# Patryk27/strolle

Hardware: AMD Instinct MI355X
Metric: Mray/s (primary + shadow + GI rays traced per second, whole job) (higher is better)
Workload: dtype f32

## Files before the change

include/strolle_hip.h:

```cpp
#ifndef STROLLE_HIP_H
#define STROLLE_HIP_H

#include <stddef.h>
#include <stdint.h>

#ifdef __cplusplus
extern "C" {
#endif

typedef struct StEngine StEngine;
typedef uint64_t StHandle;

enum StStatus {
    ST_OK = 0,
    ST_ERR_INVALID_ARGUMENT = 1,
    ST_ERR_NO_DEVICE = 2,
    ST_ERR_UNKNOWN_CAMERA = 3,
    ST_ERR_EMPTY_MESH = 4,
    ST_ERR_HIP = 5,
    ST_ERR_ATLAS_FULL = 6,
    ST_ERR_IO = 7,
    ST_ERR_PARSE = 8,
    ST_ERR_UNSUPPORTED = 9,
    ST_ERR_BVH_TOO_DEEP = 10,
// ... 400 lines not shown
int st_dist_shutdown(StEngine* e);
int st_dist_rank(StEngine* e, int* rank, int* world);
int st_dist_set_partition(StEngine* e, StHandle camera, uint32_t cols, uint32_t apron, StDistRect* owned, StDistRect* window);
int st_dist_set_grid(StEngine* e, StHandle camera, const StDistGrid* grid, uint32_t apron, StDistRect* owned, StDistRect* window);
int st_dist_gather(StEngine* e, StHandle camera, const void* frame, void* full_on_root, void* hip_stream);
int st_dist_wait(StEngine* e, StHandle camera, const void* frame, void* hip_stream, int host_wait);
int st_dist_gather_ms(StEngine* e, StHandle camera, float* ms);

enum StOutputFormat { ST_FORMAT_RGBA32F = 0, ST_FORMAT_RGBA16F = 1, ST_FORMAT_RGBA8_UNORM_SRGB = 2, ST_FORMAT_BGRA8_UNORM_SRGB = 3 };
int st_camera_set_output_format(StEngine* e, StHandle camera, int format);

typedef struct StTuning {
    uint32_t struct_size;
    uint32_t overlap;
    uint32_t fuse;
    uint32_t fuse_di_head;
    uint32_t fuse_spatial;
    uint32_t fuse_gi_sampling;
    uint32_t fuse_gi_validation;
    uint32_t fuse_gi_reprojection;
    uint32_t fuse_wavelet;
    uint32_t fuse_compose;
    uint32_t preview_both;
    uint32_t variance_in_reproject;
    uint32_t lean_frame;
    uint32_t skip_scratch_stores;
    uint32_t di_head_on_main;
    uint32_t alias_gi_history;
    uint32_t tile_map;
    uint32_t tile_map_denoise;
    int32_t side_priority;
    uint32_t staging;
    uint32_t double_buffer;
    uint32_t packed_base;
    uint32_t tick_timing;
    uint32_t anyhit_fast;
    uint32_t compact_bvh;
    uint32_t allow_deep_bvh;
    uint32_t device_bake;
    uint32_t wide_bvh;
    uint32_t wide_stack_entries;
    uint32_t primary_packets;
    uint32_t side_start;
} StTuning;
int st_engine_get_tuning(StEngine* e, StTuning* out);
int st_engine_set_tuning(StEngine* e, const StTuning* tuning);

enum StArithmetic { ST_ARITH_FAST = 0, ST_ARITH_EXACT = 1 };
int st_engine_set_arithmetic(StEngine* e, int arithmetic);
int st_engine_get_arithmetic(StEngine* e, int* out);

enum StBufferId {
    ST_BUF_PRIM_GBUFFER_D0_A = 0, ST_BUF_PRIM_GBUFFER_D0_B = 1, ST_BUF_PRIM_GBUFFER_D1_A = 2, ST_BUF_PRIM_GBUFFER_D1_B = 3,
    ST_BUF_PRIM_SURFACE_MAP_A = 4, ST_BUF_PRIM_SURFACE_MAP_B = 5, ST_BUF_REPROJECTION_MAP = 6, ST_BUF_VELOCITY_MAP = 7,
    ST_BUF_DI_RESERVOIRS_0 = 8, ST_BUF_DI_RESERVOIRS_1 = 9, ST_BUF_DI_RESERVOIRS_2 = 10,
    ST_BUF_DI_DIFF_SAMPLES = 11, ST_BUF_DI_DIFF_PREV_COLORS = 12, ST_BUF_DI_DIFF_CURR_COLORS = 13,
    ST_BUF_DI_DIFF_MOMENTS_A = 14, ST_BUF_DI_DIFF_MOMENTS_B = 15, ST_BUF_DI_DIFF_STASH = 16, ST_BUF_DI_SPEC_SAMPLES = 17,
    ST_BUF_GI_D0 = 18, ST_BUF_GI_D1 = 19, ST_BUF_GI_D2 = 20,
    ST_BUF_GI_RESERVOIRS_0 = 21, ST_BUF_GI_RESERVOIRS_1 = 22, ST_BUF_GI_RESERVOIRS_2 = 23, ST_BUF_GI_RESERVOIRS_3 = 24,
    ST_BUF_GI_DIFF_SAMPLES = 25, ST_BUF_GI_DIFF_PREV_COLORS = 26, ST_BUF_GI_DIFF_CURR_COLORS = 27,
    ST_BUF_GI_DIFF_MOMENTS_A = 28, ST_BUF_GI_DIFF_MOMENTS_B = 29, ST_BUF_GI_DIFF_STASH = 30, ST_BUF_GI_SPEC_SAMPLES = 31,
    ST_BUF_REF_HITS = 32, ST_BUF_REF_RAYS = 33, ST_BUF_REF_COLORS = 34,
    ST_BUF_DBG_USED_MEMORY = 35,
    ST_BUF_COUNT = 36
};
int st_camera_read_buffer(StEngine* e, StHandle camera, int buffer_id, void* out, size_t capacity, size_t* written);
int st_camera_write_buffer(StEngine* e, StHandle camera, int buffer_id, const void* data, size_t bytes);
int st_debug_keep_all_planes(StEngine* e, int keep);
int st_camera_buffer_stale(StEngine* e, StHandle camera, int buffer_id, int* stale);
enum StPassBit {
    ST_PASS_PRIM_VISIBILITY = 1u << 0, ST_PASS_FRAME_REPROJECTION = 1u << 1,
    ST_PASS_DI_SAMPLING = 1u << 2, ST_PASS_DI_TEMPORAL = 1u << 3, ST_PASS_DI_SPATIAL_PICK = 1u << 4, ST_PASS_DI_SPATIAL_TRACE = 1u << 5,
    ST_PASS_DI_SPATIAL_SAMPLE = 1u << 6, ST_PASS_DI_RESOLVING = 1u << 7,
    ST_PASS_GI_REPROJECTION = 1u << 8, ST_PASS_GI_SAMPLING_A = 1u << 9, ST_PASS_GI_SAMPLING_B = 1u << 10, ST_PASS_GI_TEMPORAL = 1u << 11,
    ST_PASS_GI_SPATIAL_PICK = 1u << 12, ST_PASS_GI_SPATIAL_TRACE = 1u << 13, ST_PASS_GI_SPATIAL_SAMPLE = 1u << 14,
    ST_PASS_GI_PREVIEW_0 = 1u << 15, ST_PASS_GI_PREVIEW_1 = 1u << 16, ST_PASS_GI_RESOLVING = 1u << 17,
    ST_PASS_DENOISE_REPROJECT_DI = 1u << 18, ST_PASS_DENOISE_REPROJECT_GI = 1u << 19, ST_PASS_DENOISE_VARIANCE = 1u << 20,
    ST_PASS_DENOISE_WAVELET_0 = 1u << 21,
    ST_PASS_COMPOSITION = 1u << 26, ST_PASS_BVH_HEATMAP = 1u << 27, ST_PASS_REF_TRACING = 1u << 28, ST_PASS_REF_SHADING = 1u << 29,
    ST_PASS_POST = 1u << 30
};
int st_debug_set_pass_mask(StEngine* e, uint64_t mask);
int st_debug_set_launch_filter(StEngine* e, uint64_t filter);
int st_debug_variance_flags(StEngine* e, StHandle camera, uint64_t* tile_mask_out, size_t capacity_tiles, size_t* tiles);
int st_debug_last_launches(StEngine* e, uint64_t* out_bits, size_t capacity, size_t* count);
int st_camera_ray_count(StEngine* e, StHandle camera, uint64_t* out, int reset);
int st_debug_read_scene(StEngine* e, int what, void* out, size_t capacity, size_t* written);
int st_debug_world(StEngine* e, uint32_t* light_count, uint32_t* next_frame);
int st_debug_image_rect(StEngine* e, StHandle id, uint32_t out_xywh[4]);
int st_debug_bvh_refresh(StEngine* e, uint64_t* primitives, uint64_t* reused);
int st_debug_read_lut(StEngine* e, int what, float* out, size_t capacity_floats, size_t* written_floats);

enum { ST_GLTF_OVERRIDE_REFLECTANCE = 1, ST_GLTF_OVERRIDE_PERCEPTUAL_ROUGHNESS = 2 };
typedef struct StGltfOptions {
    StHandle first_handle;
    StHandle first_image_handle;
    uint32_t override_mask;
    float reflectance;
    float perceptual_roughness;
    uint32_t subdivide;
    float light_radius;
    uint32_t _pad;
} StGltfOptions;
typedef struct StGltfSummary {
    uint32_t meshes, triangles, materials, images;
    uint32_t images_dropped;
    uint32_t primitives_skipped;
    uint32_t lights;
    uint32_t lights_skipped;
} StGltfSummary;
int st_scene_load_gltf(StEngine* e, const char* path, const StGltfOptions* options, StGltfSummary* summary);
int st_scene_load_gltf_memory(StEngine* e, const void* bytes, size_t size, const char* base_dir, const StGltfOptions* options, StGltfSummary* summary);
int st_decode_png(const void* bytes, size_t size, uint8_t* out_rgba, size_t capacity, uint32_t* width, uint32_t* height);
int st_decode_image(const void* bytes, size_t size, uint8_t* out_rgba, size_t capacity, uint32_t* width, uint32_t* height);

int st_debug_copy_bandwidth(StEngine* e, size_t bytes, int iters, double* out_gbps);

enum { ST_PROFILE_TIMING = 1, ST_PROFILE_TRAVERSAL_BYTES = 2,
       ST_PROFILE_GROUP_ATROUS = 4 ,
       ST_PROFILE_KERNEL_EVENTS = 8  };
enum { ST_PROFILE_MAX_KERNELS = 64 };
typedef struct StKernelProfile {
    char name[48];
    uint32_t launches;
    float total_ms;
    double algorithmic_bytes;
    double traversal_bytes;
} StKernelProfile;
int st_profile_enable(StEngine* e, int enabled);
int st_profile_read(StEngine* e, StKernelProfile* out, size_t capacity, size_t* count, int reset);

#ifdef __cplusplus
}
#endif
#endif
```

rust/strolle-hip/src/ffi.rs:

```rust
#![allow(non_camel_case_types, dead_code)]
use std::ffi::c_void;
use std::os::raw::c_char;

#[repr(C)]
#[derive(Clone, Copy, Default)]
pub struct StMeshTriangle {
    pub positions: [[f32; 3]; 3],
    pub normals: [[f32; 3]; 3],
    pub uvs: [[f32; 2]; 3],
    pub tangents: [[f32; 4]; 3],
}

#[repr(C)]
#[derive(Clone, Copy, Default)]
pub struct StMaterial {
    pub base_color: [f32; 4],
    pub emissive: [f32; 4],
    pub perceptual_roughness: f32,
    pub metallic: f32,
    pub reflectance: f32,
    pub ior: f32,
    pub base_color_texture: u64,
    pub emissive_texture: u64,
    pub metallic_roughness_texture: u64,
// ... 62 lines not shown
    pub alias_gi_history: u32,
    pub tile_map: u32,
    pub tile_map_denoise: u32,
    pub side_priority: i32,
    pub staging: u32,
    pub double_buffer: u32,
    pub packed_base: u32,
    pub tick_timing: u32,
    pub anyhit_fast: u32,
    pub compact_bvh: u32,
    pub allow_deep_bvh: u32,
    pub device_bake: u32,
    pub wide_bvh: u32,
    pub wide_stack_entries: u32,
    pub primary_packets: u32,
    pub side_start: u32,
}

#[repr(C)]
#[derive(Clone, Copy, PartialEq, Eq, Debug)]
pub struct StDistGrid {
    pub cols: u32,
    pub rows: u32,
    pub row_edge: [u32; 17],
    pub col_edge: [[u32; 17]; 16],
}

#[repr(C)]
#[derive(Clone, Copy, Default, PartialEq, Eq, Debug)]
pub struct StDistRect {
    pub x0: u32,
    pub y0: u32,
    pub x1: u32,
    pub y1: u32,
}

#[repr(C)]
#[derive(Clone, Copy)]
pub struct StDistUniqueId {
    pub internal: [c_char; 128],
}

pub enum StEngine {}

pub const ST_RAY_COHERENT: u32 = 1;
pub const ST_RAY_MAPPED_NORMAL: u32 = 2;

extern "C" {
    pub fn st_engine_create(device_ordinal: i32, out: *mut *mut StEngine) -> i32;
    pub fn st_engine_destroy(e: *mut StEngine);
    pub fn st_last_error() -> *const c_char;
    pub fn st_build_commit() -> *const c_char;
    pub fn st_mesh_insert(e: *mut StEngine, id: u64, triangles: *const StMeshTriangle, count: usize) -> i32;
    pub fn st_mesh_remove(e: *mut StEngine, id: u64) -> i32;
    pub fn st_material_insert(e: *mut StEngine, id: u64, material: *const StMaterial) -> i32;
    pub fn st_material_has(e: *mut StEngine, id: u64) -> i32;
    pub fn st_material_remove(e: *mut StEngine, id: u64) -> i32;
    pub fn st_image_insert_rgba8(e: *mut StEngine, id: u64, w: u32, h: u32, rgba: *const u8, srgb: i32) -> i32;
    pub fn st_image_insert_device_rgba8(e: *mut StEngine, id: u64, w: u32, h: u32, device_rgba: *const c_void, row_pitch: usize, is_dynamic: i32) -> i32;
    pub fn st_image_remove(e: *mut StEngine, id: u64) -> i32;
    pub fn st_instance_insert(e: *mut StEngine, id: u64, mesh: u64, material: u64, xform12: *const f32) -> i32;
    pub fn st_instance_remove(e: *mut StEngine, id: u64) -> i32;
    pub fn st_light_insert(e: *mut StEngine, id: u64, light: *const StLight) -> i32;
    pub fn st_light_remove(e: *mut StEngine, id: u64) -> i32;
    pub fn st_sun_update(e: *mut StEngine, azimuth: f32, altitude: f32) -> i32;
    pub fn st_camera_create(e: *mut StEngine, camera: *const StCamera, out: *mut u64) -> i32;
    pub fn st_camera_update(e: *mut StEngine, camera: u64, desc: *const StCamera) -> i32;
    pub fn st_camera_delete(e: *mut StEngine, camera: u64) -> i32;
    pub fn st_camera_set_output_format(e: *mut StEngine, camera: u64, format: i32) -> i32;
    pub fn st_tick(e: *mut StEngine, hip_stream: *mut c_void) -> i32;
    pub fn st_render_camera(e: *mut StEngine, camera: u64, out_device: *mut c_void, hip_stream: *mut c_void) -> i32;
    pub fn st_camera_present_copy(e: *mut StEngine, camera: u64, src_device: *const c_void, dst_host: *mut c_void, bytes: usize, hip_stream: *mut c_void) -> i32;
    pub fn st_camera_present_ready(e: *mut StEngine, camera: u64, dst_host: *const c_void, wait: i32, ready: *mut i32) -> i32;
    pub fn st_set_seed(e: *mut StEngine, seed: u64) -> i32;
    pub fn st_set_blue_noise(e: *mut StEngine, rgba: *const u8, bytes: usize) -> i32;
    pub fn st_engine_set_arithmetic(e: *mut StEngine, arithmetic: i32) -> i32;
    pub fn st_set_bvh_refresh(e: *mut StEngine, mode: i32) -> i32;
    pub fn st_debug_walk_overflow(e: *mut StEngine, overflows: *mut u64, wide_stack_entries: *mut u32, packets_off: *mut u32) -> i32;
    pub fn st_debug_auto_tree(e: *mut StEngine, leaf_run_weight: *mut f32, first_tree_on_device: *mut u32) -> i32;
    pub fn st_debug_device_builds(e: *mut StEngine, ticks: *mut u64) -> i32;
    pub fn st_debug_device_tree_refits(e: *mut StEngine, ticks: *mut u64) -> i32;
    pub fn st_engine_get_tuning(e: *mut StEngine, out: *mut StTuning) -> i32;
    pub fn st_engine_set_tuning(e: *mut StEngine, tuning: *const StTuning) -> i32;
    pub fn st_camera_set_window(e: *mut StEngine, camera: u64, x0: u32, y0: u32, x1: u32, y1: u32) -> i32;
    pub fn st_dist_partition(width: u32, height: u32, world: u32, cols: u32, rank: u32, owned: *mut StDistRect) -> i32;
    pub fn st_dist_window(width: u32, height: u32, owned: *const StDistRect, apron: u32, window: *mut StDistRect) -> i32;
    pub fn st_dist_unique_id(out: *mut StDistUniqueId) -> i32;
    pub fn st_dist_init(e: *mut StEngine, rank: i32, world: i32, id: *const StDistUniqueId) -> i32;
    pub fn st_dist_shutdown(e: *mut StEngine) -> i32;
    pub fn st_dist_set_partition(e: *mut StEngine, camera: u64, cols: u32, apron: u32, owned: *mut StDistRect, window: *mut StDistRect) -> i32;
    pub fn st_dist_grid(width: u32, height: u32, world: u32, cols: u32, out: *mut StDistGrid) -> i32;
    pub fn st_dist_grid_tile(grid: *const StDistGrid, rank: u32, owned: *mut StDistRect) -> i32;
    pub fn st_dist_grid_rebalance(width: u32, height: u32, current: *const StDistGrid, tile_cost: *const f32, max_step: u32, out: *mut StDistGrid) -> i32;
    pub fn st_dist_set_grid(e: *mut StEngine, camera: u64, grid: *const StDistGrid, apron: u32, owned: *mut StDistRect, window: *mut StDistRect) -> i32;
    pub fn st_dist_gather(e: *mut StEngine, camera: u64, frame: *const c_void, full_on_root: *mut c_void, hip_stream: *mut c_void) -> i32;
    pub fn st_dist_wait(e: *mut StEngine, camera: u64, frame: *const c_void, hip_stream: *mut c_void, host_wait: i32) -> i32;
}

pub const ST_ENV_KEEP_SUN: u32 = 1;
pub const ST_ENV_UNIFORM_SAMPLING: u32 = 2;
#[repr(C)]
#[derive(Clone, Copy, Debug, Default)]
pub struct StEnvironmentDesc {
    pub struct_size: u32,
    pub flags: u32,
    pub intensity: f32,
    pub yaw: f32,
}
extern "C" {
    pub fn st_environment_set(e: *mut StEngine, texels: *const f32, width: u32, height: u32, channels: u32, desc: *const StEnvironmentDesc) -> i32;
    pub fn st_environment_set_device(e: *mut StEngine, texels_device: *const c_void, width: u32, height: u32, channels: u32, row_pitch_bytes: usize, desc: *const StEnvironmentDesc) -> i32;
    pub fn st_environment_update(e: *mut StEngine, desc: *const StEnvironmentDesc) -> i32;
    pub fn st_environment_clear(e: *mut StEngine) -> i32;
    pub fn st_decode_hdr(bytes: *const c_void, size: usize, out_rgb: *mut f32, capacity_floats: usize, width: *mut u32, height: *mut u32) -> i32;
    pub fn st_debug_environment_eval(e: *mut StEngine, dirs_device: *const f32, n: u32, rgb_device: *mut f32, hip_stream: *mut c_void) -> i32;
    pub fn st_debug_environment_sample(e: *mut StEngine, u_device: *const f32 , n: u32, dir_pdf_device: *mut f32, hip_stream: *mut c_void) -> i32;
    pub fn st_debug_environment_pdf(e: *mut StEngine, dirs_device: *const f32, n: u32, pdf_device: *mut f32, hip_stream: *mut c_void) -> i32;
    pub fn st_debug_environment_sanitized(e: *mut StEngine, texels: *mut u64) -> i32;
    pub fn st_debug_environment_table(e: *mut StEngine, table: *mut c_void, capacity_bytes: usize, cells_x: *mut u32, cells_y: *mut u32) -> i32;
}

pub const ST_TONEMAP_NONE: u32 = 0;
pub const ST_TONEMAP_REINHARD: u32 = 1;
pub const ST_TONEMAP_REINHARD_LUMINANCE: u32 = 2;
pub const ST_TONEMAP_ACES_FITTED: u32 = 3;
pub const ST_TONEMAP_PBR_NEUTRAL: u32 = 4;
pub const ST_DISPLAY_AUTO_EXPOSURE: u32 = 1;
#[repr(C)]
#[derive(Clone, Copy, Debug, Default)]
pub struct StDisplayDesc {
    pub struct_size: u32,
    pub tonemap: u32,
    pub flags: u32,
    pub exposure_ev: f32,
    pub ev_min: f32,
    pub ev_max: f32,
    pub low_fraction: f32,
    pub high_fraction: f32,
    pub max_ev_step_up: f32,
    pub max_ev_step_down: f32,
}
extern "C" {
    pub fn st_camera_set_display(e: *mut StEngine, camera: u64, desc: *const StDisplayDesc) -> i32;
    pub fn st_camera_get_display(e: *mut StEngine, camera: u64, out: *mut StDisplayDesc, enabled: *mut i32) -> i32;
    pub fn st_camera_exposure(e: *mut StEngine, camera: u64, scale: *mut f32, metered_ev: *mut f32, adapted_ev: *mut f32) -> i32;
    pub fn st_debug_camera_histogram(e: *mut StEngine, camera: u64, bins: *mut u32) -> i32;
}

extern "C" {
    pub fn st_engine_set_deformation_motion(e: *mut StEngine, enabled: i32) -> i32;
    pub fn st_engine_get_deformation_motion(e: *mut StEngine, enabled: *mut i32) -> i32;
    pub fn st_engine_set_normal_mapping(e: *mut StEngine, enabled: i32) -> i32;
    pub fn st_engine_get_normal_mapping(e: *mut StEngine, enabled: *mut i32) -> i32;
    pub fn st_debug_deformation(e: *mut StEngine, instances_with_previous: *mut u64, previous_bytes: *mut u64) -> i32;
}

#[repr(C)]
#[derive(Clone, Copy, Debug, Default)]
pub struct StMorphDelta {
    pub position: [f32; 3],
    pub normal: [f32; 3],
}
extern "C" {
    pub fn st_mesh_set_morph_targets(e: *mut StEngine, mesh: u64, deltas: *const StMorphDelta, corner_count: usize, target_count: u32) -> i32;
    pub fn st_instance_set_morph_weights(e: *mut StEngine, instance: u64, weights: *const f32, target_count: u32) -> i32;
    pub fn st_debug_morphing(e: *mut StEngine, ticks: *mut u64, triangles: *mut u64, delta_bytes: *mut u64) -> i32;
// ... 272 lines not shown
```

strolle_amd/api.py:

```python
from __future__ import annotations

import ctypes as C
import dataclasses
import enum
import math
import os
import sys
from typing import Optional, Sequence

import numpy as np

_HERE = os.path.dirname(os.path.abspath(__file__))
LIB_PATH = os.environ.get("STROLLE_HIP_LIB") or os.path.join(_HERE, "csrc", "libstrolle_hip.so")
if os.environ.get("STROLLE_HIP_LIB"):
    LIB_PATH = os.environ["STROLLE_HIP_LIB"]


class StMeshTriangle(C.Structure):
    _fields_ = [("positions", C.c_float * 9), ("normals", C.c_float * 9), ("uvs", C.c_float * 6), ("tangents", C.c_float * 12)]


class StSkinVertex(C.Structure):
    _fields_ = [("joints", C.c_uint16 * 4), ("weights", C.c_float * 4)]

# ... 624 lines not shown
            self.environment_set_device = fn("environment_set_device", [vp, vp, u32, u32, u32, sz, P(StEnvironmentDesc)])
            self.environment_update = fn("environment_update", [vp, P(StEnvironmentDesc)])
            self.environment_clear = fn("environment_clear", [vp])
            self.debug_environment_eval = fn("debug_environment_eval", [vp, vp, u32, vp, vp])
            self.debug_environment_sample = fn("debug_environment_sample", [vp, vp, u32, vp, vp])
            self.debug_environment_pdf = fn("debug_environment_pdf", [vp, vp, u32, vp, vp])
            self.debug_environment_sanitized = fn("debug_environment_sanitized", [vp, P(u64)])
            self.debug_environment_table = fn("debug_environment_table", [vp, vp, sz, P(u32), P(u32)])
        if hasattr(lib, prefix + "camera_set_display"):
            self.camera_set_display = fn("camera_set_display", [vp, u64, P(StDisplayDesc)])
            self.camera_get_display = fn("camera_get_display", [vp, u64, P(StDisplayDesc), P(i32)])
            self.camera_exposure = fn("camera_exposure", [vp, u64, P(C.c_float), P(C.c_float), P(C.c_float)])
            self.debug_camera_histogram = fn("debug_camera_histogram", [vp, u64, P(u32)])
        if hasattr(lib, prefix + "camera_set_post"):
            self.camera_set_post = fn("camera_set_post", [vp, u64, P(StPostDesc)])
            self.camera_get_post = fn("camera_get_post", [vp, u64, P(StPostDesc), P(i32)])
            self.camera_output_size = fn("camera_output_size", [vp, u64, P(u32), P(u32)])
            self.post_process = fn("post_process", [vp, P(StPostDesc), vp, u32, u32, vp, i32, vp])
        if hasattr(lib, prefix + "camera_set_upscale"):
            self.camera_set_upscale = fn("camera_set_upscale", [vp, u64, P(StUpscaleDesc)])
            self.camera_get_upscale = fn("camera_get_upscale", [vp, u64, P(StUpscaleDesc), P(i32)])
            self.upscale_process = fn("upscale_process", [vp, P(StUpscaleDesc), vp, u32, u32, vp, i32, vp])
            self.debug_set_upscale_fused = fn("debug_set_upscale_fused", [vp, i32])
        if hasattr(lib, prefix + "camera_set_bloom"):
            self.camera_set_bloom = fn("camera_set_bloom", [vp, u64, P(StBloomDesc)])
            self.camera_get_bloom = fn("camera_get_bloom", [vp, u64, P(StBloomDesc), P(i32)])
            self.bloom_plan = fn("bloom_plan", [P(StBloomDesc), u32, u32, P(u32), P(u32), P(C.c_float)])
            self.debug_set_bloom_tail = fn("debug_set_bloom_tail", [vp, i32, P(u32)])
            self.bloom_process = fn("bloom_process", [vp, P(StBloomDesc), P(StDisplayDesc), vp, u32, u32, vp, i32, vp])
        if hasattr(lib, prefix + "camera_set_motion_blur"):
            self.camera_set_motion_blur = fn("camera_set_motion_blur", [vp, u64, P(StMotionBlurDesc)])
            self.camera_get_motion_blur = fn("camera_get_motion_blur", [vp, u64, P(StMotionBlurDesc), P(i32)])
            self.motion_blur_process = fn("motion_blur_process", [vp, P(StMotionBlurDesc), P(StDisplayDesc), vp, vp, vp, u32, u32, vp, i32, vp])
        if hasattr(lib, prefix + "camera_set_dof"):
            self.camera_set_dof = fn("camera_set_dof", [vp, u64, P(StDofDesc)])
            self.camera_get_dof = fn("camera_get_dof", [vp, u64, P(StDofDesc), P(i32)])
            self.dof_plan = fn("dof_plan", [P(StDofDesc), u32, u32, P(u32), P(u32), P(C.c_float)])
            self.dof_process = fn("dof_process", [vp, P(StDofDesc), P(StDisplayDesc), P(C.c_float), vp, vp, u32, u32, vp, i32, vp])
        if hasattr(lib, prefix + "camera_set_fog"):
            self.camera_set_fog = fn("camera_set_fog", [vp, u64, P(StFogDesc)])
            self.camera_get_fog = fn("camera_get_fog", [vp, u64, P(StFogDesc), P(i32)])
            self.fog_process = fn("fog_process", [vp, P(StFogDesc), P(StDisplayDesc), P(C.c_float), P(C.c_float), vp, vp, u32, u32, vp, i32, vp])
        if hasattr(lib, prefix + "camera_set_lens"):
            self.camera_set_lens = fn("camera_set_lens", [vp, u64, P(StLensDesc)])
            self.camera_get_lens = fn("camera_get_lens", [vp, u64, P(StLensDesc), P(i32)])
            self.lens_plan = fn("lens_plan", [P(StLensDesc), u32, u32, P(StLensPlan)])
            self.lens_process = fn("lens_process", [vp, P(StLensDesc), P(StDisplayDesc), vp, u32, u32, vp, i32, vp])
            self.debug_set_lens_gather = fn("debug_set_lens_gather", [vp, i32])
        if hasattr(lib, prefix + "camera_set_color_grading"):
            self.camera_set_color_grading = fn("camera_set_color_grading", [vp, u64, P(StColorGradingDesc)])
            self.camera_get_color_grading = fn("camera_get_color_grading", [vp, u64, P(StColorGradingDesc), P(i32)])
            self.color_grading_plan = fn("color_grading_plan", [P(StColorGradingDesc), P(StColorGradingPlan)])
            self.color_grading_process = fn("color_grading_process", [vp, P(StColorGradingDesc), P(StDisplayDesc), vp, u32, vp, u32, u32, vp, i32, vp])
            self.lut_insert = fn("lut_insert", [vp, u64, u32, P(C.c_float)]); self.lut_remove = fn("lut_remove", [vp, u64])
        if hasattr(lib, prefix + "camera_set_light_shafts"):
            self.camera_set_light_shafts = fn("camera_set_light_shafts", [vp, u64, P(StLightShaftsDesc)])
            self.camera_get_light_shafts = fn("camera_get_light_shafts", [vp, u64, P(StLightShaftsDesc), P(i32)])
            self.light_shafts_process = fn("light_shafts_process", [vp, P(StLightShaftsDesc), P(StDisplayDesc), P(C.c_float), P(C.c_float), vp, vp, u32, u32, vp, i32, vp])
        if hasattr(lib, prefix + "mesh_set_skin"):
            self.mesh_set_skin = fn("mesh_set_skin", [vp, u64, vp, sz, u32])
        if hasattr(lib, prefix + "mesh_set_morph_targets"):
            self.mesh_set_morph_targets = fn("mesh_set_morph_targets", [vp, u64, vp, sz, u32])
            self.instance_set_morph_weights = fn("instance_set_morph_weights", [vp, u64, P(C.c_float), u32])
            self.debug_morphing = fn("debug_morphing", [vp, P(u64), P(u64), P(u64)])
        if hasattr(lib, prefix + "engine_set_deformation_motion"):
            self.engine_set_deformation_motion = fn("engine_set_deformation_motion", [vp, i32])
            self.engine_get_deformation_motion = fn("engine_get_deformation_motion", [vp, P(i32)])
            self.debug_deformation = fn("debug_deformation", [vp, P(u64), P(u64)])
        if hasattr(lib, prefix + "engine_set_normal_mapping"):
            self.engine_set_normal_mapping = fn("engine_set_normal_mapping", [vp, i32])
            self.engine_get_normal_mapping = fn("engine_get_normal_mapping", [vp, P(i32)])
        if has_device:
            self.camera_set_rows = fn("camera_set_rows", [vp, u64, u32, u32])
            self.camera_set_output_format = fn("camera_set_output_format", [vp, u64, i32])
            self.image_insert_device_rgba8 = fn("image_insert_device_rgba8", [vp, u64, u32, u32, vp, sz, i32])
            self.debug_bvh_refresh = fn("debug_bvh_refresh", [vp, P(u64), P(u64)])
            self.scene_load_gltf = fn("scene_load_gltf", [vp, C.c_char_p, P(StGltfOptions), P(StGltfSummary)])
            self.scene_load_gltf_memory = fn("scene_load_gltf_memory", [vp, vp, sz, C.c_char_p, P(StGltfOptions), P(StGltfSummary)])
            self.decode_png = fn("decode_png", [vp, sz, vp, sz, P(u32), P(u32)])
            self.engine_set_arithmetic = fn("engine_set_arithmetic", [vp, i32]); self.engine_get_arithmetic = fn("engine_get_arithmetic", [vp, P(i32)])
            self.camera_write_buffer = fn("camera_write_buffer", [vp, u64, i32, vp, sz])
            self.debug_set_pass_mask = fn("debug_set_pass_mask", [vp, u64]); self.debug_set_launch_filter = fn("debug_set_launch_filter", [vp, u64]); self.debug_last_launches = fn("debug_last_launches", [vp, P(u64), sz, P(sz)])
            self.debug_keep_all_planes = fn("debug_keep_all_planes", [vp, i32])
            self.camera_buffer_stale = fn("camera_buffer_stale", [vp, u64, i32, P(i32)])
            self.camera_present_copy = fn("camera_present_copy", [vp, u64, vp, vp, sz, vp])
            self.camera_present_ready = fn("camera_present_ready", [vp, u64, vp, i32, P(i32)])
            if hasattr(lib, prefix + "scene_trace_rays"):
                self.scene_trace_rays = fn("scene_trace_rays", [vp, vp, u32, vp, u32, vp])
                self.scene_occluded = fn("scene_occluded", [vp, vp, u32, vp, vp])
                self.camera_pick = fn("camera_pick", [vp, u64, vp, u32, vp, vp])
                self.scene_trace_rays_host = fn("scene_trace_rays_host", [vp, vp, u32, vp])
            if hasattr(lib, prefix + "camera_render_aovs"):
                self.camera_render_aovs = fn("camera_render_aovs", [vp, u64, P(StAovTargets), vp])
            if hasattr(lib, prefix + "instance_set_pose"):
                self.instance_set_pose = fn("instance_set_pose", [vp, u64, P(C.c_float), u32])
                self.debug_skinning = fn("debug_skinning", [vp, P(u64), P(u64), P(u64)])
                self.debug_read_posed = fn("debug_read_posed", [vp, u64, P(C.c_float), sz, P(sz)])
            self.profile_enable = fn("profile_enable", [vp, i32])
            self.profile_read = fn("profile_read", [vp, P(StKernelProfile), sz, P(sz), i32])
            self.last_error = getattr(lib, prefix + "last_error"); self.last_error.restype = C.c_char_p; self.last_error.argtypes = []


_STATUS = {1: "invalid argument", 2: "no HIP device (host-only engine or HIP unavailable)", 3: "camera does not exist",
           4: "mesh contains no triangles", 5: "HIP runtime error", 6: "no more space in the atlas", 7: "file could not be read",
           8: "malformed scene file", 9: "unsupported scene file feature",
           10: "the BVH is deeper than the kernels' traversal stack (the scene was uploaded; pushes beyond 24 pending entries are dropped)",
           11: "collective transport error"}
ST_ERR_BVH_TOO_DEEP = 10


class EngineBase:

    def __init__(self, binding: _Binding, device: int = 0):
        self._b = binding
        h = C.c_void_p()
        self._check(binding.engine_create(device, C.byref(h)) if binding.has_device else binding.engine_create(C.byref(h)))
        self._h = h
        self._keep = []

    def _check(self, status: int):
        if status != 0:
            detail = ""
            if self._b.has_device:
                msg = self._b.last_error()
                detail = f": {msg.decode(errors='replace')}" if msg else ""
            raise StrolleError(f"{_STATUS.get(status, 'error')} (status {status}){detail}")

    def close(self):
        if getattr(self, "_h", None):
            self._b.engine_destroy(self._h)
            self._h = None

    def __del__(self):
        try:
            self.close()
        except Exception:
            pass

    def insert_mesh(self, handle: int, mesh: Mesh):
        data = mesh.pack()
        self._check(self._b.mesh_insert(self._h, handle, data.ctypes.data, len(data)))

    def remove_mesh(self, handle: int):
        self._check(self._b.mesh_remove(self._h, handle))

    def set_skin(self, mesh: int, joints, weights, joint_count: int):
        joints = np.asarray(joints).reshape(-1, 4); weights = np.asarray(weights, np.float32).reshape(-1, 4)
        corners = np.zeros(len(joints), SKIN_VERTEX_DTYPE)
        corners["joints"] = joints; corners["weights"] = weights
        self._check(self._b.mesh_set_skin(self._h, mesh, corners.ctypes.data if len(corners) else None, len(corners), joint_count))

    def set_morph_targets(self, mesh: int, position_deltas, normal_deltas):
        dp = np.asarray(position_deltas, np.float32); dn = np.asarray(normal_deltas, np.float32)
        if dp.ndim != 4 or dp.shape[2:] != (3, 3) or dn.shape != dp.shape:
            raise StrolleError("morph deltas: expected two arrays of shape (K, n, 3, 3)")
        deltas = np.zeros((dp.shape[0], dp.shape[1] * 3), MORPH_DELTA_DTYPE)
        deltas["position"] = dp.reshape(dp.shape[0], -1, 3); deltas["normal"] = dn.reshape(dp.shape[0], -1, 3)
        self._check(self._b.mesh_set_morph_targets(self._h, mesh, deltas.ctypes.data if deltas.size else None, deltas.shape[1], deltas.shape[0]))

    def insert_material(self, handle: int, material: Material):
        m = material.to_c()
        self._check(self._b.material_insert(self._h, handle, C.byref(m)))

    def has_material(self, handle: int) -> bool:
        return bool(self._b.material_has(self._h, handle))

# ... 120 lines not shown
    def bvh_refits(self):
        a, b = C.c_uint64(), C.c_uint64()
        self._check(self._b.debug_bvh_refits(self._h, C.byref(a), C.byref(b)))
        return a.value, b.value

    def bvh_depth(self):
        if not hasattr(self._b, "debug_bvh_depth"):
            raise StrolleError("bvh_depth() is a seam of libstrolle_hip.so (st_debug_bvh_depth); this engine's library does not export it")
        a, b = C.c_uint32(), C.c_uint32()
        self._check(self._b.debug_bvh_depth(self._h, C.byref(a), C.byref(b)))
        return a.value, b.value

    def walk_overflow(self):
        n, entries, off = C.c_uint64(), C.c_uint32(), C.c_uint32()
        self._check(self._b.debug_walk_overflow(self._h, C.byref(n), C.byref(entries), C.byref(off)))
        return n.value, entries.value, off.value

    def auto_tree(self):
        w, d = C.c_float(), C.c_uint32()
        self._check(self._b.debug_auto_tree(self._h, C.byref(w), C.byref(d)))
        return float(w.value), bool(d.value)

    def image_rect(self, handle: int):
        r = (C.c_uint32 * 4)()
        self._check(self._b.debug_image_rect(self._h, handle, r))
        return tuple(r)

    def bvh_refresh(self):
        n, r = C.c_uint64(), C.c_uint64()
        self._check(self._b.debug_bvh_refresh(self._h, C.byref(n), C.byref(r)))
        return n.value, r.value


_lib_cache = {}


def load_library(path: str = LIB_PATH) -> C.CDLL:
    if path not in _lib_cache:
        if not os.path.exists(path):
            raise StrolleError(f"{path} is missing: run `python -c 'import __graft_entry__ as g; g.build()'` (no CPU fallback exists)")
        if os.environ.get("STROLLE_HIP_PRELOAD_TORCH") == "1" and "torch" not in sys.modules:
            import torch
        _lib_cache[path] = C.CDLL(path)
    return _lib_cache[path]


def library_build_commit(path: str = LIB_PATH) -> Optional[str]:
    lib = load_library(path)
    if not hasattr(lib, "st_build_commit"):
        return None
    lib.st_build_commit.restype = C.c_char_p
    return lib.st_build_commit().decode(errors="replace")


class Engine(EngineBase):

    def __init__(self, device: int = 0, exact: Optional[bool] = None):
        super().__init__(_Binding(load_library(), "st_", True), device)
        if exact is not None:
            self.set_exact(exact)

    def set_exact(self, exact: bool):
        self._check(self._b.engine_set_arithmetic(self._h, 1 if exact else 0))

    @property
    def exact(self) -> bool:
        out = C.c_int()
        self._check(self._b.engine_get_arithmetic(self._h, C.byref(out)))
        return out.value == 1

    def write_buffer(self, camera: int, buffer: "Buffer", data: np.ndarray):
        data = np.ascontiguousarray(data)
        self._check(self._b.camera_write_buffer(self._h, camera, int(buffer), data.ctypes.data, data.nbytes))

    def keep_all_planes(self, keep: bool):
        self._check(self._b.debug_keep_all_planes(self._h, 1 if keep else 0))

    def set_pass_mask(self, mask: int):
        self._check(self._b.debug_set_pass_mask(self._h, mask & 0xFFFFFFFFFFFFFFFF))

    def set_launch_filter(self, mask: int):
        self._check(self._b.debug_set_launch_filter(self._h, mask & 0xFFFFFFFFFFFFFFFF))

    def last_launches(self):
        arr = (C.c_uint64 * 64)(); n = C.c_size_t()
        self._check(self._b.debug_last_launches(self._h, arr, 64, C.byref(n)))
        return [arr[i] for i in range(min(n.value, 64))]

    def tick(self, stream: int = 0):
        self._check(self._b.tick(self._h, stream))

    def render_camera(self, handle: int, out_device_ptr: int = 0, stream: int = 0):
        self._check(self._b.render_camera(self._h, handle, out_device_ptr, stream))

    def trace_rays(self, rays_ptr: int, count: int, hits_ptr: int, coherent: bool = False, stream: int = 0, mapped_normal: bool = False):
        flags = (RAY_COHERENT if coherent else 0) | (RAY_MAPPED_NORMAL if mapped_normal else 0)
        self._check(self._b.scene_trace_rays(self._h, rays_ptr, count, hits_ptr, flags, stream))

    def occluded(self, rays_ptr: int, count: int, out_ptr: int, stream: int = 0):
        self._check(self._b.scene_occluded(self._h, rays_ptr, count, out_ptr, stream))

    def pick(self, camera: int, pixels_ptr: int, count: int, hits_ptr: int, stream: int = 0):
        self._check(self._b.camera_pick(self._h, camera, pixels_ptr, count, hits_ptr, stream))

    def render_aovs(self, camera: int, planes: dict, stream=None):
        t = StAovTargets(); t.struct_size = C.sizeof(StAovTargets)
        for k, v in planes.items():
            k = Aov(k)
            if v is None:
                continue
            if hasattr(v, "data_ptr"):
                scalar, comps = AOV_ELEMENT[k]
                per_pixel = v.shape[-1] if comps > 1 and v.dim() > 0 else comps
                if not v.is_contiguous() or v.element_size() != np.dtype(scalar).itemsize or per_pixel != comps:
                    raise StrolleError(f"AOV plane {k.name}: expected a contiguous tensor of {comps} x {np.dtype(scalar).name} per pixel")
                v = v.data_ptr()
            t.planes[int(k)] = int(v)
        if stream is not None and hasattr(stream, "cuda_stream"):
            stream = stream.cuda_stream
        self._check(self._b.camera_render_aovs(self._h, camera, C.byref(t), stream or 0))

    def set_pose(self, instance: int, matrices):
        if matrices is None:
            self._check(self._b.instance_set_pose(self._h, instance, None, 0)); return
        m = np.asarray(matrices, np.float32).reshape(-1, 3, 4)
        flat = np.ascontiguousarray(m.transpose(0, 2, 1).reshape(-1), dtype=np.float32)
        self._check(self._b.instance_set_pose(self._h, instance, flat.ctypes.data_as(C.POINTER(C.c_float)), len(m)))

    def set_morph_weights(self, instance: int, weights):
        if weights is None:
            self._check(self._b.instance_set_morph_weights(self._h, instance, None, 0)); return
        w = np.ascontiguousarray(np.asarray(weights, np.float32).reshape(-1))
        self._check(self._b.instance_set_morph_weights(self._h, instance, w.ctypes.data_as(C.POINTER(C.c_float)), len(w)))

    def morphing_stats(self):
        a, b, c = C.c_uint64(), C.c_uint64(), C.c_uint64()
        self._check(self._b.debug_morphing(self._h, C.byref(a), C.byref(b), C.byref(c)))
        return a.value, b.value, c.value

    def skinning_stats(self):
        a, b, c = C.c_uint64(), C.c_uint64(), C.c_uint64()
        self._check(self._b.debug_skinning(self._h, C.byref(a), C.byref(b), C.byref(c)))
        return a.value, b.value, c.value

    def read_posed(self, instance: int) -> np.ndarray:
        n = C.c_size_t()
        self._check(self._b.debug_read_posed(self._h, instance, None, 0, C.byref(n)))
        out = np.zeros(n.value, np.float32)
        self._check(self._b.debug_read_posed(self._h, instance, out.ctypes.data_as(C.POINTER(C.c_float)), n.value, C.byref(n)))
        return out.reshape(-1, 24)

    def set_deformation_motion(self, enabled: bool):
        self._check(self._b.engine_set_deformation_motion(self._h, 1 if enabled else 0))

    @property
    def deformation_motion(self) -> bool:
        on = C.c_int()
        self._check(self._b.engine_get_deformation_motion(self._h, C.byref(on)))
        return bool(on.value)

    def set_normal_mapping(self, enabled: bool):
        self._check(self._b.engine_set_normal_mapping(self._h, 1 if enabled else 0))

    def get_normal_mapping(self) -> bool:
        on = C.c_int()
        self._check(self._b.engine_get_normal_mapping(self._h, C.byref(on)))
# ... 461 lines not shown
```

strolle_amd/csrc/k_common.h:

```cpp
#pragma once
#include "st_device.h"
#include "st_passes.h"
#include "st_kernels.h"

namespace st {

constexpr int kBlockThreads = 256;
#ifdef ST_MIN_WAVES
#define ST_KERNEL_BOUNDS __launch_bounds__(kBlockThreads, ST_MIN_WAVES)
#else
#define ST_KERNEL_BOUNDS __launch_bounds__(kBlockThreads)
#endif
#define ST_STACK_LDS(SE, name) extern __shared__ __align__(16) unsigned char st_stack_lds_[]; SE* name = reinterpret_cast<SE*>(st_stack_lds_)
inline uint32_t stack_lds_bytes(const KArgs& a, size_t slot_bytes) { return a.stack_entries * (uint32_t)kBlockThreads * (uint32_t)slot_bytes; }

struct TileWindow { uint32_t tx0, tx1, ty0, ty1; };
__host__ __device__ inline TileWindow tile_window(const KArgs& a, bool half_x) {
    uint32_t tiles_x = (a.width + 7u) >> 3;
    if (half_x) tiles_x >>= 1;
    const uint32_t shift = half_x ? 4u : 3u, round = half_x ? 15u : 7u;
    TileWindow w;
    w.tx0 = a.col0 >> shift;
    w.tx1 = (a.col1 + round) >> shift; if (w.tx1 > tiles_x) w.tx1 = tiles_x;
    if (w.tx0 > w.tx1) w.tx0 = w.tx1;
    w.ty0 = a.row0 >> 3;
    w.ty1 = (a.row1 + 7u) >> 3;
    return w;
}
struct LaunchDims { uint32_t tiles_x, tile_x0, tile_y0, tile_y1, blocks; };
inline LaunchDims launch_dims(const KArgs& a, bool half_x) {
    const TileWindow w = tile_window(a, half_x);
    LaunchDims d;
    d.tiles_x = w.tx1 - w.tx0; d.tile_x0 = w.tx0;
    d.tile_y0 = w.ty0; d.tile_y1 = w.ty1;
    const uint32_t groups_x = (d.tiles_x + 3u) / 4u;
    d.blocks = groups_x * (d.tile_y1 - d.tile_y0);
    return d;
}

ST_D TileCoord resolve_tile(const KArgs& a, bool half_x) {
    const TileWindow w = tile_window(a, half_x);
    TileCoord tc = tile_for_thread(w.tx1 - w.tx0, w.ty1 - w.ty0, a.tile_map);
    tc.x += w.tx0; tc.y += w.ty0;
    return tc;
}
ST_D bool resolve_gid_of_block(const KArgs& a, bool half_x, uint32_t b, U2* gid) {
    const TileWindow w = tile_window(a, half_x);
    TileCoord tc = tile_for_block(b, w.tx1 - w.tx0, w.ty1 - w.ty0, a.tile_map);
    tc.x += w.tx0; tc.y += w.ty0;
    if (!tc.valid) return false;
    *gid = pixel_in_tile(tc);
    return true;
}
ST_D bool resolve_gid(const KArgs& a, bool half_x, U2* gid) {
    const TileCoord tc = resolve_tile(a, half_x);
    if (!tc.valid) return false;
    *gid = pixel_in_tile(tc);
    return true;
}
ST_D bool owns_pixel(const KArgs& a, U2 p) { return p.x < a.width && p.y < a.height && p.y >= a.row0 && p.y < a.row1 && p.x >= a.col0 && p.x < a.col1; }

constexpr uint32_t kStack16Texels = 4u * 65536u;
inline uint32_t stack16_limit(const KArgs& a) {
    if (a.bvh_w) return a.bvh_w_links16 ? 0xffffffffu : 0u;
    return a.bvh_c ? kStack16Texels / 2u : kStack16Texels;
}
#ifdef ST_NO_LDS_SCENE
inline bool scene_fits_lds(const KArgs&) { return false; }
#else
inline bool scene_fits_lds(const KArgs& a) { return a.bvh_len > 0u && a.bvh_len <= kLdsSceneTexels; }
#endif
#define ST_SCENE_PROLOGUE                                                                                                        \
    __shared__ float4 s_scene_bvh_[LDS_SCENE ? kLdsSceneTexels : 1];                                                             \
    __shared__ GpuLight s_lights_[kLdsLights];                                                                                   \
    KArgs a = a_in;                                                                                                              \
    {                                                                                                                            \
        const uint32_t n_l_ = (a_in.n_lights_buf < kLdsLights ? a_in.n_lights_buf : kLdsLights) * 7u;                            \
        for (uint32_t i_ = threadIdx.x; i_ < n_l_; i_ += kBlockThreads)                                                          \
            reinterpret_cast<float4*>(s_lights_)[i_] = reinterpret_cast<const float4*>(a_in.lights)[i_];                         \
        if (LDS_SCENE) for (uint32_t i_ = threadIdx.x; i_ < a_in.bvh_len; i_ += kBlockThreads) s_scene_bvh_[i_] = a_in.bvh[i_];  \
        __syncthreads();                                                                                                         \
        a.lights_lds = s_lights_;                                                                                                \
        if (LDS_SCENE) a.bvh = s_scene_bvh_;                                                                                     \
    }
#define ST_QUERY_PROLOGUE                                                                                            \
    __shared__ float4 s_scene_bvh_[LDS_SCENE ? kLdsSceneTexels : 1];                                                 \
    KArgs a = a_in;                                                                                                  \
    if (LDS_SCENE) {                                                                                                 \
        for (uint32_t i_ = threadIdx.x; i_ < a_in.bvh_len; i_ += kBlockThreads) s_scene_bvh_[i_] = a_in.bvh[i_];     \
        __syncthreads();                                                                                             \
        a.bvh = s_scene_bvh_;                                                                                        \
    }
#define ST_SCENE_PROLOGUE_WITH_BYTE_TABLES                                                                                       \
    __shared__ float s_byte_luts_[kByteLutFloats];                                                                               \
    for (uint32_t i_ = threadIdx.x; i_ < kByteLutFloats / 4u; i_ += kBlockThreads)                                               \
        reinterpret_cast<float4*>(s_byte_luts_)[i_] = reinterpret_cast<const float4*>(a_in.byte_luts)[i_];                       \
    ST_SCENE_PROLOGUE                                                                                                            \
    a.byte_luts = s_byte_luts_;
#define ST_TRACE_FLAGS_(...) , ##__VA_ARGS__
#define ST_TRACE_KERNEL_(k, lds, flags, se) (k<lds ST_TRACE_FLAGS_ flags, se>)
#define ST_LAUNCH_TRACE(kernel_tmpl, flags, half, stream, ...)                                                                                                      \
    do {                                                                                                                                                            \
        if (scene_fits_lds(a)) ST_LAUNCH_SMEM(ST_TRACE_KERNEL_(kernel_tmpl, true, flags, uint16_t), half, stack_lds_bytes(a, 2), stream, __VA_ARGS__);              \
        else if (a.bvh_len < stack16_limit(a)) ST_LAUNCH_SMEM(ST_TRACE_KERNEL_(kernel_tmpl, false, flags, uint16_t), half, stack_lds_bytes(a, 2), stream, __VA_ARGS__); \
        else ST_LAUNCH_SMEM(ST_TRACE_KERNEL_(kernel_tmpl, false, flags, uint32_t), half, stack_lds_bytes(a, 4), stream, __VA_ARGS__);                               \
    } while (0)

#define ST_LAUNCH_SMEM(kernel, half, smem, stream, ...)                                                          \
    do {                                                                                                         \
        const LaunchDims d_ = launch_dims(a, half);                                                              \
        if (d_.blocks) ST_KLAUNCH_SMEM(kernel, dim3(d_.blocks), dim3(kBlockThreads), smem, stream, __VA_ARGS__); \
// ... 9 lines not shown
```

strolle_amd/csrc/k_denoise.hip:

```cpp
#include "k_common.h"

namespace st {
namespace ST_KNS {


struct f2 { float x, y; };
struct i2v { int x, y; };
ST_D f2 mk2(float x, float y) { f2 r; r.x = x; r.y = y; return r; }
ST_D f2 operator+(f2 a, f2 b) { return mk2(a.x + b.x, a.y + b.y); }
ST_D f2 operator-(f2 a, f2 b) { return mk2(a.x - b.x, a.y - b.y); }
ST_D f2 operator*(f2 a, f2 b) { return mk2(a.x * b.x, a.y * b.y); }
ST_D f2 operator*(f2 a, float b) { return mk2(a.x * b, a.y * b); }
ST_D f2 operator*(float a, f2 b) { return mk2(a * b.x, a * b.y); }
ST_D f2 operator+(f2 a, float b) { return mk2(a.x + b, a.y + b); }
ST_D f2 operator-(f2 a) { return mk2(-a.x, -a.y); }
ST_D f2 splat2(float x) { return mk2(x, x); }
ST_D f2 sqrt2(f2 x) { return mk2(fsqrt(x.x), fsqrt(x.y)); }
ST_D float div_by(float x, float d, float inv_d) {
#if ST_FAST_DEVICE
    return x * inv_d;
#else
    return x / d;
#endif
}
// ... 91 lines not shown
    if (a.variance_in_reproject && !slow) return;
    if (!mine) return;
    if (csn.w == 0.0f) { di_out[center] = cdi; gi_out[center] = cgi; return; }
    float di_var, gi_var;
    if (!slow) {
        di_var = cdi_m.z - sqr(cdi_m.y);
        gi_var = cgi_m.z - sqr(cgi_m.y);
    } else {
        variance_short_history(csn, cdi, cgi, s_sn, s_l, ((int)(pos.y & 7u) + 2) * PITCH + (int)(wave * 8u + (pos.x & 7u)) + 3, PITCH, &di_var, &gi_var);
    }
    di_var = fmax_(di_var, 0.0f);
    gi_var = fmax_(gi_var, 0.0f);
    if (a.variance_in_reproject) {
        reinterpret_cast<float*>(&di_out[center])[3] = di_var;
        reinterpret_cast<float*>(&gi_out[center])[3] = gi_var;
        return;
    }
    di_out[center] = f4(xyz(cdi), di_var);
    gi_out[center] = f4(xyz(cgi), gi_var);
}

struct WaveletCenter {
    float4 sn; V3 n; f2 sqrt_luma, luma_sigma; float leeway, inv_leeway;
    f2 sum_w, sum_r, sum_g, sum_b, sum_v;
};
ST_D f2 sqrt_luma2(float4 di, float4 gi) { return sqrt2((mk2(di.x, gi.x) * 0.2126f + mk2(di.y, gi.y) * 0.7152f) + mk2(di.z, gi.z) * 0.0722f); }
ST_D WaveletCenter wavelet_begin(float4 csn, float4 cdi, float4 cgi, float strength, f2 c_sqrt_luma) {
    WaveletCenter c;
    c.sn = csn; c.n = v3(csn.x, csn.y, csn.z);
    c.sqrt_luma = c_sqrt_luma;
    c.luma_sigma = mk2(lerpf(2.5f, 0.5f, fsqrt(cdi.w)), lerpf(1.0f, 0.0f, fsqrt(cgi.w)));
    c.leeway = csn.w * (0.33f / strength); c.inv_leeway = frcp(c.leeway);
    c.sum_w = splat2(1.0f); c.sum_r = mk2(cdi.x, cgi.x); c.sum_g = mk2(cdi.y, cgi.y); c.sum_b = mk2(cdi.z, cgi.z); c.sum_v = mk2(cdi.w, cgi.w);
    return c;
}
ST_D bool wavelet_shared(const WaveletCenter& c, float4 ssn, float* depth_weight, float* normal_weight) {
    if (ssn.w == 0.0f) return false;
    const float diff = fabsf(ssn.w - c.sn.w);
    *depth_weight = diff >= c.leeway ? 0.0f : 1.0f - div_by(diff, c.leeway, c.inv_leeway);
    *normal_weight = pow64_(fmax_(dot(v3(ssn.x, ssn.y, ssn.z), c.n), 0.0f));
    return !(*depth_weight == 0.0f || *normal_weight == 0.0f);
}
ST_D void wavelet_tap(WaveletCenter& c, float4 sdi, float4 sgi, f2 t_sqrt_luma, float depth_weight, float normal_weight) {
    const f2 r = mk2(sdi.x, sgi.x), g = mk2(sdi.y, sgi.y), b = mk2(sdi.z, sgi.z), v = mk2(sdi.w, sgi.w);
    const f2 d = c.sqrt_luma - t_sqrt_luma;
    const f2 luma_weight = mk2(fabsf(d.x), fabsf(d.y)) * c.luma_sigma;
    const f2 w = exp_pair(-luma_weight) * depth_weight * normal_weight;
    if (w.x > 0.0f && w.y > 0.0f) {
        c.sum_w = c.sum_w + w; c.sum_r = c.sum_r + w * r; c.sum_g = c.sum_g + w * g; c.sum_b = c.sum_b + w * b; c.sum_v = c.sum_v + (w * w) * v;
    } else {
        if (w.x > 0.0f) { c.sum_w.x += w.x; c.sum_r.x += w.x * r.x; c.sum_g.x += w.x * g.x; c.sum_b.x += w.x * b.x; c.sum_v.x += (w.x * w.x) * v.x; }
        if (w.y > 0.0f) { c.sum_w.y += w.y; c.sum_r.y += w.y * r.y; c.sum_g.y += w.y * g.y; c.sum_b.y += w.y * b.y; c.sum_v.y += (w.y * w.y) * v.y; }
    }
}
struct WaveletOut { float4 di, gi; bool lit; };
ST_D WaveletOut wavelet_end(const WaveletCenter& c) {
    const f2 ww = c.sum_w * c.sum_w;
    WaveletOut o;
    o.di = wavelet_resolve(c.sum_r.x, c.sum_g.x, c.sum_b.x, c.sum_v.x, c.sum_w.x, ww.x);
    o.gi = wavelet_resolve(c.sum_r.y, c.sum_g.y, c.sum_b.y, c.sum_v.y, c.sum_w.y, ww.y);
    o.lit = true;
    return o;
}
template <int S, int P>
ST_D WaveletOut wavelet_pixel_lds(const float4* s_sn, const float4* s_di, const float4* s_gi, int lc, float strength) {
    const float4 csn = s_sn[lc], cdi = s_di[lc], cgi = s_gi[lc];
    if (csn.w == 0.0f) { WaveletOut o; o.di = cdi; o.gi = cgi; o.lit = false; return o; }
    WaveletCenter c = wavelet_begin(csn, cdi, cgi, strength, sqrt_luma2(cdi, cgi));
#pragma unroll
    for (int t = 0; t < 8; t++) {
        const int k = t < 4 ? t : t + 1, ox = k % 3 - 1, oy = k / 3 - 1;
        const int lt = lc + oy * S * P + ox * S;
        float dw, nw;
        if (!wavelet_shared(c, s_sn[lt], &dw, &nw)) continue;
        const float4 tdi = s_di[lt], tgi = s_gi[lt];
        wavelet_tap(c, tdi, tgi, sqrt_luma2(tdi, tgi), dw, nw);
    }
    return wavelet_end(c);
}

constexpr int kWvW = 32, kWvH = 16, kWvThreads = kWvW * kWvH;
struct WaveletBlock { int32_t x0, y0; bool valid; };
__host__ __device__ inline void wavelet_grid(const KArgs& a, uint32_t bw, uint32_t* bx0, uint32_t* groups_x, uint32_t* rows) {
    const uint32_t c1 = a.col1 < a.width ? a.col1 : a.width;
    *bx0 = a.col0 / bw;
    const uint32_t bx1 = (c1 + bw - 1u) / bw;
    *groups_x = bx1 > *bx0 ? bx1 - *bx0 : 0u;
    const uint32_t ty0 = a.row0 >> 3, ty1 = (a.row1 + 7u) >> 3;
    *rows = ((ty1 - ty0) * 8u + kWvH - 1u) / kWvH;
}
template <int BW = kWvW>
ST_D WaveletBlock wavelet_block(const KArgs& a) {
    uint32_t bx0, groups_x, rows;
    wavelet_grid(a, BW, &bx0, &groups_x, &rows);
    const uint32_t ty0 = a.row0 >> 3;
    const uint32_t n_blocks = groups_x * rows, b = blockIdx.x;
    uint32_t lin = b;
    if (a.tile_map == 0u) {
        const uint32_t q = n_blocks >> 3, r = n_blocks & 7u, xcd = b & 7u, k = b >> 3;
        lin = (xcd < r ? xcd * (q + 1u) : r * (q + 1u) + (xcd - r) * q) + k;
    } else if (a.tile_map == 2u) {
        const uint32_t chunk = groups_x * 2u * 8u, full = (n_blocks / chunk) * chunk;
        if (b < full) { const uint32_t c = b / chunk, i = b - c * chunk; lin = c * chunk + (i & 7u) * (groups_x * 2u) + (i >> 3); }
    }
    WaveletBlock w;
    const uint32_t gy = lin / groups_x, gx = lin - gy * groups_x;
    w.x0 = (int32_t)((bx0 + gx) * BW); w.y0 = (int32_t)(ty0 * 8u + gy * kWvH);
    w.valid = gy < rows;
    return w;
}
inline uint32_t wavelet_blocks(const KArgs& a, uint32_t block_w = kWvW) {
    uint32_t bx0, groups_x, rows;
    wavelet_grid(a, block_w, &bx0, &groups_x, &rows);
    return groups_x * rows;
}
ST_D bool wavelet_owns(const KArgs& a, int32_t px, int32_t py) { return px >= 0 && py >= 0 && owns_pixel(a, u2((uint32_t)px, (uint32_t)py)); }

void launch_denoise_variance(const KArgs& a, float4* di_out, float4* gi_out, hipStream_t s) { ST_LAUNCH(k_denoise_variance, false, s, a, di_out, gi_out); }

template <int HALO, int P, int BW = kWvW>
ST_D void wavelet_stage(const KArgs& a, const WaveletBlock& blk, const float4* di_in, const float4* gi_in, float4* s_sn, float4* s_di, float4* s_gi) {
    constexpr int WW = BW + 2 * HALO, WH = kWvH + 2 * HALO;
    for (int i = (int)threadIdx.x; i < WW * WH; i += kWvThreads) {
        const int ry = i / WW, rx = i - ry * WW;
        const int32_t gx = blk.x0 - HALO + rx, gy = blk.y0 - HALO + ry;
        const int li = ry * P + rx;
        if (gx >= 0 && gy >= 0 && gx < (int32_t)a.width && gy < (int32_t)a.height) {
            const uint32_t at = (uint32_t)gy * a.width + (uint32_t)gx;
            const float4 tsn = a.sn[at], tdi = di_in[at], tgi = gi_in[at];
            s_sn[li] = tsn; s_di[li] = tdi; s_gi[li] = tgi;
        } else {
            s_sn[li] = f4z();
        }
    }
}

__global__ __launch_bounds__(kWvThreads) void k_denoise_wavelet_12(const KArgs a, float strength0, float strength1, const float4* di_in, float4* di_mid, float4* di_out,
                                                                   const float4* gi_in, float4* gi_mid, float4* gi_out) {
    constexpr int HALO = 3, WW = kWvW + 2 * HALO, WH = kWvH + 2 * HALO, P = 38;
    constexpr int RW = kWvW + 4, RH = kWvH + 4;
    __shared__ float4 s_sn[P * WH];
    __shared__ float4 s_di[P * WH];
    __shared__ float4 s_gi[P * WH];
    const WaveletBlock blk = wavelet_block(a);
    if (!blk.valid) return;
    wavelet_stage<HALO, P>(a, blk, di_in, gi_in, s_sn, s_di, s_gi);
    __syncthreads();
    float4 r_di[2], r_gi[2]; int r_at[2];
#pragma unroll
    for (int it = 0; it < 2; it++) {
        const int idx = (int)threadIdx.x + it * kWvThreads;
        r_at[it] = -1;
        if (idx >= RW * RH) continue;
        const int ry = idx / RW, rx = idx - ry * RW;
        const int lc = (ry + 1) * P + rx + 1;
        r_at[it] = lc;
        const WaveletOut o = wavelet_pixel_lds<1, P>(s_sn, s_di, s_gi, lc, strength0);
        r_di[it] = o.di; r_gi[it] = o.gi;
        const bool lit = o.lit;
        const int32_t px = blk.x0 - 2 + rx, py = blk.y0 - 2 + ry;
        if (rx >= 2 && rx < 2 + kWvW && ry >= 2 && ry < 2 + kWvH && wavelet_owns(a, px, py)) {
            const uint32_t center = (uint32_t)py * a.width + (uint32_t)px;
            di_mid[center] = r_di[it];
            if (lit) gi_mid[center] = r_gi[it];
        }
    }
    __syncthreads();
#pragma unroll
    for (int it = 0; it < 2; it++) if (r_at[it] >= 0) {
        s_di[r_at[it]] = r_di[it]; s_gi[r_at[it]] = r_gi[it];
    }
    __syncthreads();
    const int x = (int)(threadIdx.x & 31u), y = (int)(threadIdx.x >> 5);
    const int32_t px = blk.x0 + x, py = blk.y0 + y;
    if (!wavelet_owns(a, px, py)) return;
    const uint32_t center = (uint32_t)py * a.width + (uint32_t)px;
    const WaveletOut o = wavelet_pixel_lds<2, P>(s_sn, s_di, s_gi, (y + HALO) * P + x + HALO, strength1);
    di_out[center] = o.di;
    gi_out[center] = o.gi;
}

template <int S>
__global__ __launch_bounds__(kWvThreads) void k_denoise_wavelet_lds(const KArgs a, float strength, const float4* di_in, float4* di_out, const float4* gi_in, float4* gi_out) {
    constexpr int WH = kWvH + 2 * S, P = (kWvW + 2 * S + 7) / 16 * 16 + 8;
    static_assert(P >= kWvW + 2 * S && P % 16 == 8, "pitch");
    __shared__ float4 s_sn[P * WH];
    __shared__ float4 s_di[P * WH];
// ... 144 lines not shown
```

strolle_amd/csrc/st_abi.cpp:

```cpp
#include "st_engine.h"

using namespace st;
static Engine* E(StEngine* e) { return reinterpret_cast<Engine*>(e); }
#define ST_REQUIRE(cond, msg) do { if (!(cond)) return fail(ST_ERR_INVALID_ARGUMENT, msg); } while (0)
#define ST_CAMERA(c, e, h)                                                                                        \
    const auto c##_it = E(e)->cameras.find(h);                                                                    \
    if (c##_it == E(e)->cameras.end()) return fail(ST_ERR_UNKNOWN_CAMERA, "camera does not exist");               \
    CameraState& c = *c##_it->second

template <class Desc> static int camera_set(StEngine* e, StHandle h, int (Engine::*set)(CameraState&, const Desc*), const Desc* desc) {
    ST_REQUIRE(e, "null engine");
    ST_CAMERA(cam, e, h);
    return (E(e)->*set)(cam, desc);
}
template <class Desc, int N> static int camera_get(StEngine* e, StHandle h, NodeSetting<Desc, N> CameraState::*setting, Desc* out, int* enabled) {
    ST_REQUIRE(e, "null engine");
    ST_CAMERA(cam, e, h);
    const NodeSetting<Desc, N>& s = cam.*setting;
    if (out) { *out = s.desc; out->struct_size = sizeof(Desc); }
    if (enabled) *enabled = s.on ? 1 : 0;
    return ST_OK;
}

extern "C" {
// ... 407 lines not shown
    E(e)->blue_noise.assign(rgba, rgba + bytes); E(e)->blue_noise_dirty = true;
    return ST_OK;
}
int st_debug_read_lut(StEngine* e, int what, float* out, size_t capacity_floats, size_t* written_floats) {
    ST_REQUIRE(e && what >= 0 && what < 3, "bad lut id");
    Engine* en = E(e);
    if (!en->has_device) return fail(ST_ERR_NO_DEVICE, "host-only engine has no LUTs");
    const size_t n[3] = {256 * 64 * 4, 32 * 32 * 4, 256 * 256 * 4};
    const DeviceArray* src[3] = {&en->d_transmittance, &en->d_scattering, &en->d_sky};
    if (written_floats) *written_floats = n[what];
    if (!out) return ST_OK;
    ST_REQUIRE(capacity_floats >= n[what], "buffer too small");
    ST_HIP(hipSetDevice(en->device));
    ST_HIP(hipDeviceSynchronize());
    ST_HIP(hipMemcpy(out, src[what]->ptr, n[what] * sizeof(float), hipMemcpyDeviceToHost));
    return ST_OK;
}

int st_camera_read_buffer(StEngine* e, StHandle h, int id, void* out, size_t capacity, size_t* written) {
    ST_REQUIRE(e && id >= 0 && id < ST_BUF_COUNT, "bad buffer id");
    Engine* en = E(e);
    ST_CAMERA(c, e, h);
    if (!en->has_device) return fail(ST_ERR_NO_DEVICE, "host-only engine has no camera buffers");
    if (written) *written = c.plane_bytes[id];
    if (!out) return ST_OK;
    ST_REQUIRE(capacity >= c.plane_bytes[id], "buffer too small");
    ST_HIP(hipSetDevice(en->device));
    ST_HIP(hipDeviceSynchronize());
    const float4* src = (id == ST_BUF_GI_RESERVOIRS_1 && c.gi_aliased) ? c.plane[ST_BUF_GI_RESERVOIRS_0] : c.plane[id];
    ST_HIP(hipMemcpy(out, src, c.plane_bytes[id], hipMemcpyDeviceToHost));
    return ST_OK;
}
int st_camera_buffer_stale(StEngine* e, StHandle h, int id, int* stale) {
    ST_REQUIRE(e && stale && id >= 0 && id < ST_BUF_COUNT, "bad argument");
    ST_CAMERA(c, e, h);
    const uint32_t lean = c.last_lean;
    bool s = false;
    if (lean & kLeanPrim) s |= (id == ST_BUF_VELOCITY_MAP && !(lean & kLeanKeepVelocity)) || id == ST_BUF_PRIM_SURFACE_MAP_A || id == ST_BUF_PRIM_SURFACE_MAP_B;
    if (lean & kLeanSamples) s |= id == ST_BUF_DI_DIFF_SAMPLES || id == ST_BUF_GI_DIFF_SAMPLES;
    if (lean & kLeanGiRes2) s |= id == ST_BUF_GI_RESERVOIRS_2;
    if (lean & kLeanGiMid) s |= id == ST_BUF_GI_RESERVOIRS_3;
    if (c.last_lean_composed) s |= id == ST_BUF_DI_DIFF_CURR_COLORS || id == ST_BUF_GI_DIFF_CURR_COLORS;
    *stale = s ? 1 : 0;
    return ST_OK;
}
int st_camera_write_buffer(StEngine* e, StHandle h, int id, const void* data, size_t bytes) {
    ST_REQUIRE(e && data && id >= 0 && id < ST_BUF_COUNT, "bad buffer id");
    Engine* en = E(e);
    ST_CAMERA(c, e, h);
    if (!en->has_device) return fail(ST_ERR_NO_DEVICE, "host-only engine has no camera buffers");
    ST_REQUIRE(bytes == c.plane_bytes[id], "size does not match the buffer");
    ST_HIP(hipSetDevice(en->device));
    ST_HIP(hipDeviceSynchronize());
    { const int rc = materialize_gi_history(c); if (rc) return rc; }
    ST_HIP(hipMemcpy(c.plane[id], data, bytes, hipMemcpyHostToDevice));
    if (id == ST_BUF_PRIM_SURFACE_MAP_A) c.surface_map_replaced[0] = true;
    if (id == ST_BUF_PRIM_SURFACE_MAP_B) c.surface_map_replaced[1] = true;
    return ST_OK;
}
int st_debug_variance_flags(StEngine* e, StHandle h, uint64_t* tile_mask_out, size_t capacity_tiles, size_t* tiles) {
    ST_REQUIRE(e && tiles, "null argument");
    Engine* en = E(e);
    ST_CAMERA(c, e, h);
    if (!en->has_device) return fail(ST_ERR_NO_DEVICE, "host-only engine");
    *tiles = c.tile_mask_tiles();
    if (!tile_mask_out) return ST_OK;
    ST_REQUIRE(capacity_tiles >= c.tile_mask_tiles(), "buffer too small");
    ST_HIP(hipSetDevice(en->device)); ST_HIP(hipDeviceSynchronize());
    ST_HIP(hipMemcpy(tile_mask_out, c.tile_mask.ptr, c.tile_mask_tiles() * sizeof(uint64_t), hipMemcpyDeviceToHost));
    return ST_OK;
}
int st_debug_set_pass_mask(StEngine* e, uint64_t mask) {
    ST_REQUIRE(e, "null engine");
    Engine* en = E(e);
    if (en->has_device) { ST_HIP(hipSetDevice(en->device)); for (auto& kv : en->cameras) { const int rc = materialize_gi_history(*kv.second); if (rc) return rc; } }
    en->pass_mask = mask;
    return ST_OK;
}
int st_debug_set_launch_filter(StEngine* e, uint64_t filter) {
    ST_REQUIRE(e, "null engine");
    E(e)->launch_filter = filter;
    return ST_OK;
}
int st_debug_last_launches(StEngine* e, uint64_t* out_bits, size_t capacity, size_t* count) {
    ST_REQUIRE(e && count, "null argument");
    const std::vector<uint64_t>& v = E(e)->last_launches;
    *count = v.size();
    for (size_t i = 0; i < v.size() && i < capacity && out_bits; i++) out_bits[i] = v[i];
    return ST_OK;
}
int st_engine_set_arithmetic(StEngine* e, int arithmetic) {
    ST_REQUIRE(e, "null engine");
    ST_REQUIRE(arithmetic == ST_ARITH_FAST || arithmetic == ST_ARITH_EXACT, "unknown arithmetic");
    Engine* en = E(e);
    if (en->arithmetic == arithmetic) return ST_OK;
    en->arithmetic = arithmetic;
    en->L = arithmetic == ST_ARITH_EXACT ? launchers_exact() : launchers_fast();
    if (en->has_device) {
        ST_HIP(hipSetDevice(en->device));
        ST_HIP(hipDeviceSynchronize());
        en->L.launch_build_byte_luts(static_cast<float*>(en->d_byte_luts.ptr), nullptr);
        ST_HIP(hipDeviceSynchronize());
        en->atmosphere_initialized = false; en->sky_known = false;
    }
    return ST_OK;
}
int st_engine_get_tuning(StEngine* e, StTuning* out) { ST_REQUIRE(e && out, "null argument"); *out = E(e)->tuning; return ST_OK; }
int st_engine_set_tuning(StEngine* e, const StTuning* t) { ST_REQUIRE(e && t, "null argument"); return E(e)->set_tuning(*t); }
int st_engine_get_arithmetic(StEngine* e, int* out) { ST_REQUIRE(e && out, "null argument"); *out = E(e)->arithmetic; return ST_OK; }
int st_camera_ray_count(StEngine* e, StHandle h, uint64_t* out, int reset) {
    ST_REQUIRE(e && out, "null argument");
    Engine* en = E(e);
    ST_CAMERA(cam, e, h);
    if (!en->has_device) return fail(ST_ERR_NO_DEVICE, "host-only engine");
    unsigned long long host[2 * KS_COUNT];
    ST_HIP(hipSetDevice(en->device));
    ST_HIP(hipDeviceSynchronize());
    { const int rc2 = read_counters(cam, host); if (rc2) return rc2; }
    uint64_t total = 0;
    for (int i = 0; i < KS_COUNT; i++) total += host[2 * i];
    *out = total;
    if (reset) { ST_HIP(hipMemset(cam.counters.ptr, 0, kCounterBytes)); memset(cam.profiled_traversal_bytes, 0, sizeof(cam.profiled_traversal_bytes)); ST_HIP(hipDeviceSynchronize()); }
    return ST_OK;
}
int st_debug_read_scene(StEngine* e, int what, void* out, size_t capacity, size_t* written) {
    ST_REQUIRE(e, "null engine");
    Engine* en = E(e);
    const void* p; size_t bytes;
    if (SceneTree::debug_reads(what)) {
        if (int rc = en->tree.debug_read(what, &p, &bytes)) return rc;
    } else {
        if (what == 1 && en->instances.any_host_stale()) en->bake_stale_on_host();
        if (int rc = en->take_deferred_status()) return rc;
        switch (what) {
            case 1: p = en->slots.triangles().data(); bytes = en->slots.size() * sizeof(HostTriangle); break;
            case 2: p = en->lights.table().data(); bytes = en->lights.table().size() * sizeof(GpuLight); break;
            case 3: p = en->materials.gpu().data(); bytes = en->materials.gpu().size() * sizeof(GpuMaterial); break;
            default: return fail(ST_ERR_INVALID_ARGUMENT, "unknown scene buffer");
        }
    }
    if (written) *written = bytes;
    if (!out) return ST_OK;
    ST_REQUIRE(capacity >= bytes, "buffer too small");
    if (bytes) memcpy(out, p, bytes);
    return ST_OK;
}
int st_debug_world(StEngine* e, uint32_t* light_count, uint32_t* next_frame) {
    ST_REQUIRE(e && light_count && next_frame, "null argument");
    *light_count = E(e)->lights.count(); *next_frame = E(e)->frame;
    return ST_OK;
}

int st_set_bvh_refresh(StEngine* e, int mode) {
    ST_REQUIRE(e, "null engine");
    ST_REQUIRE(mode == ST_BVH_REBUILD || mode == ST_BVH_REFIT || mode == ST_BVH_REFIT_DEVICE || mode == ST_BVH_BUILD_DEVICE || mode == ST_BVH_AUTO, "unknown refresh mode");
    E(e)->tree.set_refresh_mode(mode);
    return ST_OK;
}
int st_debug_device_builds(StEngine* e, uint64_t* ticks) { ST_REQUIRE(e && ticks, "null argument"); *ticks = E(e)->tree.device_build_ticks(); return ST_OK; }
int st_debug_device_tree_refits(StEngine* e, uint64_t* ticks) { ST_REQUIRE(e && ticks, "null argument"); *ticks = E(e)->tree.device_tree_refit_ticks(); return ST_OK; }
int st_debug_bvh_depth(StEngine* e, uint32_t* deepest_internal_chain, uint32_t* stack_entries) {
    ST_REQUIRE(e && deepest_internal_chain && stack_entries, "null argument");
    E(e)->tree.depth(deepest_internal_chain, stack_entries);
    return ST_OK;
}
int st_debug_walk_overflow(StEngine* e, uint64_t* overflows, uint32_t* wide_stack_entries, uint32_t* packets_off) {
// ... 96 lines not shown
```

strolle_amd/csrc/st_device.h:

```cpp
#pragma once
#include "st_types.h"

namespace st {

#define ST_D __device__ __forceinline__

struct TileCoord { uint32_t x, y; bool valid; };
ST_D TileCoord tile_for_block(uint32_t b, uint32_t tiles_x, uint32_t tiles_y, uint32_t map_mode) {
    const uint32_t groups_x = (tiles_x + 3u) >> 2;
    const uint32_t n_blocks = groups_x * tiles_y;
    uint32_t lin = b;
    if (map_mode == 0u) {
        const uint32_t q = n_blocks >> 3, r = n_blocks & 7u;
        const uint32_t xcd = b & 7u, k = b >> 3;
        lin = (xcd < r ? xcd * (q + 1u) : r * (q + 1u) + (xcd - r) * q) + k;
    } else if (map_mode == 2u) {
        const uint32_t chunk = groups_x * 4u * 8u;
        const uint32_t full = (n_blocks / chunk) * chunk;
        if (b < full) {
            const uint32_t c = b / chunk, i = b - c * chunk;
            const uint32_t xcd = i & 7u, k = i >> 3;
            lin = c * chunk + xcd * (groups_x * 4u) + k;
        }
    }
    const uint32_t wave = threadIdx.x >> 6;
    TileCoord t;
    t.y = lin / groups_x;
    t.x = (lin - t.y * groups_x) * 4u + wave;
    t.valid = b < n_blocks && t.x < tiles_x && t.y < tiles_y;
    return t;
}
ST_D TileCoord tile_for_thread(uint32_t tiles_x, uint32_t tiles_y, uint32_t map_mode) { return tile_for_block(blockIdx.x, tiles_x, tiles_y, map_mode); }
ST_D U2 pixel_in_tile(TileCoord t) {
    const uint32_t lane = threadIdx.x & 63u;
    return u2(t.x * 8u + (lane & 7u), t.y * 8u + (lane >> 3));
}
template <class SE>
ST_D SE* lane_stack(const KArgs& a, SE* lds) { return lds + (threadIdx.x >> 6) * (a.stack_entries * 64u) + (threadIdx.x & 63u); }

ST_D void count_rays_n(const KArgs& a, uint32_t rays , unsigned long long used_memory) {
    unsigned long long* line = a.ray_counter + (blockIdx.x & (kCounterLines - 1u)) * 8u;
    if (rays & 1u) atomicAdd(line, 1ull);
    if (rays & 2u) atomicAdd(line, 2ull);
    if (a.count_bytes) atomicAdd(line + 1, used_memory);
}
ST_D void count_rays_many(const KArgs& a, uint32_t rays, unsigned long long used_memory) {
    unsigned long long* line = a.ray_counter + (blockIdx.x & (kCounterLines - 1u)) * 8u;
    atomicAdd(line, (unsigned long long)rays);
    if (a.count_bytes) atomicAdd(line + 1, used_memory);
}
ST_D void count_rays(const KArgs& a, uint32_t used_memory) {
    unsigned long long* line = a.ray_counter + (blockIdx.x & (kCounterLines - 1u)) * 8u;
    atomicAdd(line, 1ull);
    if (a.count_bytes) atomicAdd(line + 1, (unsigned long long)used_memory);
}

ST_D uint32_t u32_from_bytes(uint32_t a, uint32_t b, uint32_t c, uint32_t d) { return a | (b << 8) | (c << 16) | (d << 24); }
ST_D U2 resolve_checkerboard(U2 gid, uint32_t frame) { return u2(gid.x * 2u + ((frame + gid.y) % 2u), gid.y); }
ST_D U2 resolve_checkerboard_alt(U2 gid, uint32_t frame) { return resolve_checkerboard(gid, frame + 1u); }
ST_D bool got_checkerboard_at(U2 p, uint32_t frame) { U2 q = resolve_checkerboard(u2(p.x / 2u, p.y), frame); return q.x == p.x && q.y == p.y; }

ST_D V2 normal_encode(V3 n) {
    n = n / (fabsf(n.x) + fabsf(n.y) + fabsf(n.z));
    V2 r;
    if (n.z >= 0.0f) r = v2(n.x, n.y);
    else { r = v2(copysignf(1.0f - fabsf(n.y), n.x), copysignf(1.0f - fabsf(n.x), n.y)); }
    return r * 0.5f + 0.5f;
}
ST_D V3 normal_decode(V2 e) {
    e = e * 2.0f - 1.0f;
    V3 n = v3(e.x, e.y, 1.0f - fabsf(e.x) - fabsf(e.y));
    const float t = fmax_(-n.z, 0.0f);
    n.x -= copysignf(t, n.x);
    n.y -= copysignf(t, n.y);
    return normalize(n);
}

struct WhiteNoise {
    uint32_t state;
    ST_D uint32_t sample_int() {
        state = state * 747796405u + 2891336453u;
        const uint32_t word = ((state >> ((state >> 28) + 4u)) ^ state) * 277803737u;
        return (word >> 22) ^ word;
    }
    ST_D float sample() { return (float)sample_int() * 2.3283064365386963e-10f; }
    ST_D V2 sample_circle() { const float angle = sample() * kPi * 2.0f; float s, c; sincos_(angle, &s, &c); return v2(c, s); }
    ST_D V2 sample_disk() { const float radius = fsqrt(sample()); return sample_circle() * radius; }
    ST_D V3 sample_sphere() {
        const float phi = sample() * 2.0f * kPi;
        const float cos_theta = sample() * 2.0f - 1.0f;
        const float u = sample();
        const float theta = acos_(cos_theta);
        const float r = fsqrt(u);
        float st_, ct_, sp_, cp_;
        sincos_(theta, &st_, &ct_); sincos_(phi, &sp_, &cp_);
        return v3(r * st_ * cp_, r * st_ * sp_, r * ct_);
    }
    ST_D V3 sample_hemisphere(V3 normal) {
        const float cos_theta = sample();
        const float sin_theta = fsqrt(1.0f - sqr(cos_theta));
        const float phi = 2.0f * kPi * sample();
        V3 t, b;
        any_orthonormal_pair(normal, &t, &b);
        float sp_, cp_;
#if defined(ST_ABL_HEMI_POLY)
        sincos_poly_(phi, &sp_, &cp_);
#else
// ... 759 lines not shown
```

strolle_amd/csrc/st_engine.cpp:

```cpp
#include "st_engine.h"

namespace st {

thread_local std::string g_last_error;
thread_local LaunchEvents g_launch_events;

StTuning default_tuning() {
    StTuning t{};
    t.struct_size = sizeof(StTuning);
    t.overlap = t.fuse = t.fuse_di_head = t.fuse_spatial = t.fuse_gi_sampling = t.fuse_gi_validation = t.fuse_gi_reprojection = 1u;
    t.fuse_wavelet = t.fuse_compose = t.preview_both = t.variance_in_reproject = t.lean_frame = 1u;
    t.skip_scratch_stores = t.di_head_on_main = t.alias_gi_history = 1u;
    t.tile_map = 1u; t.tile_map_denoise = 2u; t.side_priority = 0;
    t.staging = t.double_buffer = t.packed_base = 1u; t.tick_timing = 0u;
    t.anyhit_fast = 1u; t.compact_bvh = 1u; t.wide_bvh = 1u; t.primary_packets = 1u;
    t.allow_deep_bvh = 0u; t.device_bake = 1u;
    t.side_start = 2u;
    return t;
}
static void tuning_from_environment(StTuning& t) {
    struct Clear { const char* name; uint32_t StTuning::*field; };
    static const Clear clears[] = {
        {"ST_NO_OVERLAP", &StTuning::overlap}, {"ST_NO_FUSE", &StTuning::fuse}, {"ST_NO_FUSE_DI_HEAD", &StTuning::fuse_di_head},
        {"ST_NO_FUSE_SPATIAL", &StTuning::fuse_spatial}, {"ST_NO_FUSE_GI_SAMPLING", &StTuning::fuse_gi_sampling},
        {"ST_NO_FUSE_GI_VALIDATION", &StTuning::fuse_gi_validation}, {"ST_NO_FUSE_GI_REPROJECTION", &StTuning::fuse_gi_reprojection},
        {"ST_NO_FUSE_WAVELET", &StTuning::fuse_wavelet}, {"ST_NO_FUSE_COMPOSE", &StTuning::fuse_compose}, {"ST_NO_PREVIEW_BOTH", &StTuning::preview_both},
        {"ST_NO_VARIANCE_IN_REPROJECT", &StTuning::variance_in_reproject},
        {"ST_KEEP_ALL_PLANES", &StTuning::lean_frame}, {"ST_KEEP_SCRATCH", &StTuning::skip_scratch_stores}, {"ST_NO_GI_ALIAS", &StTuning::alias_gi_history},
        {"ST_NO_STAGING", &StTuning::staging}, {"ST_NO_DOUBLE_BUFFER", &StTuning::double_buffer}, {"ST_NO_PACKED_BASE", &StTuning::packed_base},
        {"ST_NO_ANYHIT_FAST", &StTuning::anyhit_fast}, {"ST_NO_COMPACT_BVH", &StTuning::compact_bvh}, {"ST_NO_WIDE_BVH", &StTuning::wide_bvh}, {"ST_NO_PRIMARY_PACKETS", &StTuning::primary_packets},
    };
    for (const Clear& c : clears) if (const char* v = getenv(c.name)) { if (atoi(v) != 0) t.*c.field = 0u; else if (t.*c.field == 0u) t.*c.field = 1u; }
    struct Value { const char* name; uint32_t StTuning::*field; };
    static const Value values[] = {
        {"ST_DI_HEAD_ON_MAIN", &StTuning::di_head_on_main}, {"ST_TILE_MAP_DENOISE", &StTuning::tile_map_denoise}, {"ST_TICK_TIMING", &StTuning::tick_timing},
        {"ST_ALLOW_DEEP_BVH", &StTuning::allow_deep_bvh}, {"ST_DEVICE_BAKE", &StTuning::device_bake}, {"ST_SIDE_START", &StTuning::side_start},
    };
    if (const char* v = getenv("ST_TILE_MAP")) t.tile_map = t.tile_map_denoise = (uint32_t)atoi(v);
    for (const Value& c : values) if (const char* v = getenv(c.name)) t.*c.field = (uint32_t)atoi(v);
    if (const char* v = getenv("ST_SIDE_PRIORITY")) t.side_priority = atoi(v);
}

Engine::Engine() {
    blue_noise.assign(256 * 256 * 4, 0);
    reset_profile_totals();
    tuning = default_tuning();
    tuning_from_environment(tuning);
    staging.enabled = tuning.staging != 0u;
    if (const char* x = getenv("ST_BLOOM_TAIL_BYTES")) bloom_tail_wanted = atoi(x);
    if (const char* x = getenv("ST_UPSCALE_FUSED")) upscale_fused = (uint32_t)atoi(x) <= 3u ? (uint32_t)atoi(x) : 0u;
    if (const char* x = getenv("ST_EXP")) exp_flags = (uint32_t)strtoul(x, nullptr, 0);
    if (const char* ex = getenv("ST_EXACT")) if (atoi(ex) != 0) { arithmetic = ST_ARITH_EXACT; L = launchers_exact(); }
}
int Engine::set_tuning(const StTuning& t) {
    if (t.struct_size != sizeof(StTuning)) return fail(ST_ERR_INVALID_ARGUMENT, "StTuning::struct_size does not match this library");
    if (t.tile_map > 2u || t.tile_map_denoise > 2u) return fail(ST_ERR_INVALID_ARGUMENT, "tile_map is 0, 1 or 2");
    if (t.side_start > 3u) return fail(ST_ERR_INVALID_ARGUMENT, "side_start is 0 ... 3");
    if (t.wide_stack_entries != 0u && (t.wide_stack_entries < 8u || t.wide_stack_entries > 56u)) return fail(ST_ERR_INVALID_ARGUMENT, "wide_stack_entries is 0 (default) or 8 ... 56");
    if (t.wide_stack_entries != tuning.wide_stack_entries) wide_stack_rearmed = 0u;
    tuning = t;
    staging.enabled = tuning.staging != 0u;
    return ST_OK;
}
void Engine::note_walk_overflow() {
    const bool lane = walk_flags_host[0] != 0u, packet = walk_flags_host[1] != 0u;
    walk_flags_host[0] = 0u; walk_flags_host[1] = 0u;
    if (!lane && !packet) return;
    walk_overflows++; walk_overflow_unreported = true;
    if (packet) packets_overflowed = true;
    if (lane) {
        const uint32_t now = wide_stack_entries_now();
        wide_stack_rearmed = now < 32u ? 32u : (now < 48u ? 48u : 56u);
    }
}
void Engine::reset_profile_totals() {
    for (int i = 0; i < KS_COUNT; i++) {
        memset(&profile_totals[i], 0, sizeof(StKernelProfile));
        snprintf(profile_totals[i].name, sizeof(profile_totals[i].name), "%s", kernel_info(i).name);
    }
}

Engine::~Engine() {
    release_dist();
    if (!has_device) return;
    (void)hipSetDevice(device);
    (void)hipDeviceSynchronize();
}

}
```

strolle_amd/csrc/st_engine.h:

```cpp
#pragma once
#include <algorithm>
#include <cstdio>
#include <chrono>
#include <cmath>
#include <cstring>
#include <initializer_list>
#include <map>
#include <memory>
#include <string>
#include <unordered_map>
#include <vector>

#include "../../include/strolle_hip.h"
#include "st_lbvh.h"
#include "st_atlas.h"
#include "st_bvh.h"
#include "st_kernels.h"
#include "st_ranges.h"

#include <thread>

namespace st {

extern thread_local std::string g_last_error;
// ... 314 lines not shown
inline int materialize_gi_history(CameraState& c) {
    if (!c.gi_aliased) return ST_OK;
    ST_HIP(hipDeviceSynchronize());
    ST_HIP(hipMemcpy(c.plane[ST_BUF_GI_RESERVOIRS_1], c.plane[ST_BUF_GI_RESERVOIRS_0], c.plane_bytes[ST_BUF_GI_RESERVOIRS_0], hipMemcpyDeviceToDevice));
    c.gi_aliased = false;
    return ST_OK;
}
inline int read_counters(const CameraState& c, unsigned long long* host ) {
    std::vector<unsigned long long> raw(kCounterWordsPerSlot * KS_COUNT);
    hipError_t err = hipMemcpy(raw.data(), c.counters.ptr, kCounterBytes, hipMemcpyDeviceToHost);
    if (err != hipSuccess) return fail(ST_ERR_HIP, std::string("hipMemcpy(counters): ") + hipGetErrorString(err));
    for (int s = 0; s < KS_COUNT; s++) {
        unsigned long long rays = 0, bytes = 0;
        for (uint32_t l = 0; l < kCounterLines; l++) { rays += raw[(size_t)s * kCounterWordsPerSlot + l * 8]; bytes += raw[(size_t)s * kCounterWordsPerSlot + l * 8 + 1]; }
        host[2 * s] = rays; host[2 * s + 1] = bytes;
    }
    return ST_OK;
}


struct ProfileRecord { int slot; hipEvent_t start, stop; double bytes; uint32_t launches; bool owns_start; };

StTuning default_tuning();
struct DistState;
int dist_partition(uint32_t width, uint32_t height, uint32_t world, uint32_t cols, uint32_t rank, StDistRect* owned);
int dist_window(uint32_t width, uint32_t height, const StDistRect* owned, uint32_t apron, StDistRect* window);
int dist_grid(uint32_t width, uint32_t height, uint32_t world, uint32_t cols, StDistGrid* out);
int dist_grid_tile(const StDistGrid* g, uint32_t rank, StDistRect* owned);
int dist_grid_rebalance(uint32_t width, uint32_t height, const StDistGrid* cur, const float* cost, uint32_t max_step, StDistGrid* out);

struct Engine {
    int device = -1;
    bool has_device = false;
    uint64_t base_seed = 0;
    uint32_t frame = 1;

    MeshStore meshes; MaterialStore materials; ImageAtlas images; LightStore lights; InstanceStore instances; TriangleSlots slots;
    bool moved_on_device = false;
    bool materials_changed_this_tick = false;
    uint64_t device_bakes = 0, device_baked_triangles = 0;
    void bake_stale_on_host();

    Deformer deform{*this};
    int deferred_status = ST_OK;
    int take_deferred_status() { const int rc = deferred_status; deferred_status = ST_OK; return rc; }

    SceneTree tree{*this};

    StagingRing staging;

    bool sync_every_tick = false;
    float sun_azimuth = 0.0f, sun_altitude = 0.35f; bool sun_dirty = true;
    V3 sun_dir_ = v3s(0.0f);

    std::vector<uint8_t> blue_noise; bool blue_noise_dirty = true;
    bool atmosphere_initialized = false, sky_known = false; float known_sun_altitude = 0.0f;

    SceneCopies copies{*this};
    struct EnvMap { DeviceArray texels, table; uint32_t w = 0, h = 0, gw = 0, gh = 0; Fence fence; };
    enum EnvEditKind { ENV_EDIT_NONE, ENV_EDIT_HOST, ENV_EDIT_DEVICE, ENV_EDIT_CLEAR };
    struct EnvEdit { EnvEditKind kind = ENV_EDIT_NONE; std::vector<float4> texels; const void* src = nullptr; size_t pitch = 0; uint32_t w = 0, h = 0, channels = 0; };
    EnvEdit env_edit;
    StEnvironmentDesc env_desc{}, env_desc_next{};
    bool env_set = false, env_sun_off = false;
    std::unique_ptr<EnvMap> env_live; Retired<EnvMap> env_retired{copies};
    DeviceArray d_env_grid, d_env_bad ; uint64_t env_sanitized = 0;
    std::vector<float> env_grid_host; std::vector<EnvCell> env_table_host;

    struct Lut { DeviceArray texels; uint32_t size = 0; Fence fence; };
    struct LutEdit { uint32_t size = 0; std::vector<float4> texels; };
    std::map<StHandle, LutEdit> lut_edits;
    std::map<StHandle, std::unique_ptr<Lut>> luts_live; Retired<Lut> luts_retired{copies};

    DeviceArray d_byte_luts, d_atlas, d_blue_noise, d_transmittance, d_scattering, d_sky;

    std::unordered_map<uint64_t, std::unique_ptr<CameraState>> cameras; uint64_t next_camera = 0;

    int arithmetic = ST_ARITH_FAST;
    Launchers L = launchers_fast();
    std::vector<uint64_t> last_launches;
    uint64_t launch_filter = ~0ull;
    uint64_t pass_mask = ~0ull;
    StTuning tuning;
    uint32_t exp_flags = 0;
    bool profiling = false;
    bool count_bytes = false;
    bool profile_kernel_events = false;
    bool profile_group_atrous = false;
    std::vector<ProfileRecord> profile_records;
    std::vector<Event> profile_events; std::vector<hipEvent_t> event_pool;
    StKernelProfile profile_totals[KS_COUNT];

    Engine();
    int set_tuning(const StTuning& t);
    DistState* dist = nullptr;
    void release_dist();
    void dist_forget_camera(uint64_t handle);
    int dist_set_partition(uint64_t handle, CameraState& c, uint32_t cols, uint32_t apron);
    int dist_set_grid(uint64_t handle, CameraState& c, const StDistGrid& grid, uint32_t apron);
    int dist_gather(uint64_t handle, CameraState& c, const void* frame, void* full, hipStream_t stream);
    int dist_wait(uint64_t handle, const void* frame, hipStream_t stream, bool host);
    void dist_guard(uint64_t handle, const void* out, hipStream_t s);
    int dist_gather_ms(uint64_t handle, float* ms);
    void reset_profile_totals();
    ~Engine();
    static void release_camera(CameraState& c);
    int present_copy(CameraState& c, const void* src, void* dst, size_t bytes, hipStream_t stream);
    int present_ready(CameraState& c, const void* dst, int wait, int* ready);

    void insert_mesh(uint64_t id, const StMeshTriangle* t, size_t count);
    void remove_mesh(uint64_t id);
    void insert_instance(uint64_t id, uint64_t mesh, uint64_t material, const Affine& x);
    void remove_instance(uint64_t id);

    void drop_instance_triangles(uint64_t id);
    struct BakeJob { const std::vector<StMeshTriangle>* mesh; const InstanceRec* inst; uint32_t material; size_t first, count; };
    bool refresh_instances();
    void bake_jobs_on_host(const std::vector<BakeJob>& jobs, size_t total);
    int bake_on_device(SceneSet& t, hipStream_t up, bool* pageable);

    bool wide_only_tuning() const { return arithmetic == ST_ARITH_FAST && tuning.wide_bvh && tuning.compact_bvh && tuning.anyhit_fast && !count_bytes; }
    bool heatmap_camera() const { for (const auto& kv : cameras) if (kv.second->desc.mode == ST_MODE_BVH_HEATMAP) return true; return false; }
    PinnedBuffer walk_flags_mem; volatile uint32_t* walk_flags_host = nullptr; uint32_t* walk_flags_dev = nullptr;
    uint32_t wide_stack_rearmed = 0u;
    bool packets_overflowed = false;
    uint64_t walk_overflows = 0; bool walk_overflow_unreported = false;
    uint32_t wide_stack_entries_now() const { return wide_stack_rearmed ? wide_stack_rearmed : (tuning.wide_stack_entries ? tuning.wide_stack_entries : (uint32_t)kBvhStackSize); }
    void note_walk_overflow();
    enum TriArrays : unsigned { TRI_GEO = 1u , TRI_ATTR = 2u  };
    bool tri_fits(const SceneSet& t, unsigned arrays) const;
    int upload_tri_slots(SceneSet& t, unsigned arrays, bool whole, hipStream_t up, bool* pageable);
    int tick(hipStream_t stream);
    TreePlan refresh_scene();
    void refresh_sun_and_lights();
    void apply_environment();
    int upload_environment(TickIo& io);
    void environment_args(KArgs& a) const;
    int environment_debug(uint32_t what, const float* in, uint32_t n, float* out, hipStream_t stream);
    int upload_scene(TreePlan plan, TickIo& io);
    int upload_images(TickIo& io);
    int upload_lights(TickIo& io);
    int report_deep_bvh();

    static GpuCamera serialize_camera(const StCamera& c);
    int allocate_camera(CameraState& c);

    hipEvent_t take_event();
    struct OpenScope { int slot = -1; hipStream_t stream = nullptr; hipEvent_t start{}; bool owns_start = true; double bytes = 0; uint32_t launches = 0; } open_scope;
    void profile_begin(int slot, hipStream_t s, double bytes);
    hipEvent_t profile_close();
    int drain_profile();

    static void present_guard(CameraState& c, const void* out, hipStream_t s) {
        for (auto& p : c.present) if (p.pending && p.src == out) (void)p.ev_done.wait(s);
    }

    int render(CameraState& c, void* out, hipStream_t stream);
    int set_display(CameraState& c, const StDisplayDesc* desc);
    int display_begin(CameraState& c, hipStream_t stream, bool heatmap, DisplayArgs& d);
    int display_finalize(CameraState& c, hipStream_t stream);
    int display_exposure(CameraState& c, float* scale, float* metered_ev, float* adapted_ev);
    int display_histogram(CameraState& c, uint32_t* bins);
    struct PostPlan { bool fxaa = false, resample = false; PostArgs fx{}, rs{}; double fxaa_bytes = 0.0, resample_bytes = 0.0; };
    static PostPlan post_plan(const StPostDesc& d, bool fxaa, const void* src, uint32_t w, uint32_t h, void* mid, void* dst, uint32_t format);
    int set_post(CameraState& c, const StPostDesc* desc);
    int post_process(const StPostDesc* desc, const void* src, uint32_t w, uint32_t h, void* dst, int format, hipStream_t stream);
// ... 86 lines not shown
```

strolle_amd/csrc/st_render.cpp:

```cpp
#include "st_engine.h"

namespace st {

void Engine::release_camera(CameraState& c) {
    c.slab.release(); c.counters.release(); c.tile_mask.release();
    c.side_stream.reset();
    for (Event* e : {&c.ev_di_head, &c.ev_gi_done, &c.ev_prim_ok, &c.ev_frame_done, &c.ev_setup, &c.ev_lds_done}) e->reset();
    c.have_prev_frame_events = c.have_lds_done = false;
    c.join_present(); c.present_stream.reset();
    for (auto& p : c.present) p = CameraState::PresentSlot();
}

int Engine::present_copy(CameraState& c, const void* src, void* dst, size_t bytes, hipStream_t stream) {
    if (!has_device) return fail(ST_ERR_NO_DEVICE, "present copy on a host-only engine");
    ST_HIP(hipSetDevice(device));
    if (!c.present_stream) ST_HIP(hipStreamCreateWithFlags(&c.present_stream.h, hipStreamNonBlocking));
    CameraState::PresentSlot* slot = nullptr;
    for (auto& p : c.present) if (p.dst == dst) slot = &p;
    if (!slot) { slot = &c.present[c.present_next & 1u]; c.present_next++; }
    if (slot->pending) ST_HIP(hipEventSynchronize(slot->ev_done.h));
    slot->src = src; slot->dst = dst;
    if (int rc = slot->ev_src.record(stream)) return rc;
    if (int rc = slot->ev_src.wait(c.present_stream)) return rc;
    ST_HIP(hipMemcpyAsync(dst, src, bytes, hipMemcpyDeviceToHost, c.present_stream));
// ... 56 lines not shown
}

int Engine::normal_map_geo(hipStream_t stream, bool flagged, const float4** geo) {
    *geo = nullptr;
    const std::vector<float4>& tri_geo = slots.geo();
    if (!(normal_mapping || flagged) || !materials.any_normal_map || tri_geo.empty()) return ST_OK;
    SceneSet& scene = copies.scene.current();
    if (!scene.geo_current) {
        const size_t bytes = tri_geo.size() * sizeof(float4);
        if (int rc = scene.tri_geo.reserve(bytes, std::max<size_t>(bytes * 3 / 2, 4096))) return rc;
        ST_HIP(hipMemcpyAsync(scene.tri_geo.ptr, tri_geo.data(), bytes, hipMemcpyHostToDevice, stream));
        ST_HIP(hipStreamSynchronize(stream));
        scene.geo_current = true;
    }
    if (scene.tri_geo.capacity < tri_geo.size() * sizeof(float4)) return fail(ST_ERR_INVALID_ARGUMENT, "normal mapping: the live scene copy's hit-test records are short of the scene's triangle slots");
    *geo = static_cast<const float4*>(scene.tri_geo.ptr);
    return ST_OK;
}
int Engine::scene_args(KArgs& a, bool heatmap) const {
    const SceneSet& scene = copies.scene.current();
    a.tri_attr = static_cast<const float4*>(scene.tri_attr.ptr); a.instance_xforms = static_cast<const float4*>(scene.xforms.ptr);
    a.materials = static_cast<const GpuMaterial*>(scene.materials.ptr); a.material_base_packed = tuning.packed_base ? static_cast<const uint32_t*>(scene.base_packed.ptr) : nullptr;
    a.atlas = static_cast<const uchar4*>(d_atlas.ptr); a.byte_luts = static_cast<const float*>(d_byte_luts.ptr);
    a.tri_slots = (uint32_t)slots.size();
    a.count_bytes = count_bytes ? 1u : 0u;
    a.exp_flags = exp_flags;
    if (int rc = tree.walk_args(scene.tree, a, heatmap)) return rc;
    a.walk_flags = walk_flags_dev;
    a.anyhit_contract = (count_bytes || !tuning.anyhit_fast) ? 1u : 0u;
    a.atlas_w = images.width(); a.atlas_h = images.height();
    return ST_OK;
}
void Engine::light_args(KArgs& a) const {
    a.lights = static_cast<const GpuLight*>(copies.lights.current().buf.ptr);
    a.blue_noise = static_cast<const uchar4*>(d_blue_noise.ptr);
    a.transmittance_lut = static_cast<const float4*>(d_transmittance.ptr); a.sky_lut = static_cast<const float4*>(d_sky.ptr);
    a.n_lights_buf = (uint32_t)lights.table().size(); a.light_count = lights.count();
    a.sun_altitude = sun_altitude; a.sun_dir[0] = sun_dir_.x; a.sun_dir[1] = sun_dir_.y; a.sun_dir[2] = sun_dir_.z;
    environment_args(a);
}

namespace {
enum HdrNode { kNodeFog, kNodeShafts, kNodeDof, kNodeMBlur, kNodeBloom, kNodeLens, kNodeGrade, kHdrNodes };
struct HdrNodeRow { uint32_t early; bool reads_depth, reads_velocity; };
constexpr HdrNodeRow kHdrNode[kHdrNodes] = {
           {0u, true, false},
                                  {0u, true, false},
               {1u, false, false},
          {1u, false, true},
                    {0u, false, false},
       {0u, false, false},
      {0u, false, false},
};
struct HdrWork {
    Engine::ShaftsPlan shafts_plan; Engine::DofPlan dof_plan; Engine::MBlurPlan mblur_plan; Engine::BloomPlan bloom_plan; Engine::GradePlan grade_plan; StLensPlan lens_plan;
    Engine::Lut* grade_lut = nullptr;
    Engine::GradeStep grade; Engine::LensStep lens; Engine::FogStep fog; Engine::ShaftsSteps shafts; Engine::DofSteps dof; Engine::MBlurSteps mblur; Engine::BloomSteps bloom;
};
struct OutputRoute {
    bool post_fxaa = false, post = false, keep_velocity = false ;
    bool up_steps = false , up_nearest = false ;
    void* hdr_plane[kHdrNodes] = {};
    Fence* planes_read[kHdrNodes] = {};
    bool on(int n) const { return hdr_plane[n] != nullptr; }
    NodeTarget target(int n) const {
        for (int k = n + 1; k < kHdrNodes; k++) if (hdr_plane[k]) return {hdr_plane[k], frame_format, true, frame_disp};
        return {frame_out, frame_format, false, frame_disp};
    }
    void* comp_out = nullptr; uint32_t comp_format = 0; DisplayArgs comp_disp{};
    void* frame_out = nullptr; uint32_t frame_format = 0; DisplayArgs frame_disp{};
};
struct FrameSwitches {
    bool needs_di, needs_gi, denoise, any_objects, tracing, whole_graph, gi_runs, swap_gi_history, gi_preview_both, even_tiles, compose_in_wavelet;
    bool fuse_gi_validation_now, fuse_gi_reprojection_now, two_streams;
    uint32_t gi_source, lean, variance_in_reproject, skip_dead_scratch, gi_skip_history_copy;
};
struct Frame {
    Engine& e; CameraState& c; void* const out; const hipStream_t stream; hipStream_t cur;
    const float4* nm_tri_geo = nullptr;
    KArgs a{}; OutputRoute route; FrameSwitches s{}; HdrWork work;
    const uint32_t mode, pseed;
    bool mask_split = false, di_reprojected = false, gi_reprojected = false, composed = false, luts_generated_now = false; uint32_t launch_ordinal = 0u;
    int side_rc = ST_OK;
    Frame(Engine& e_, CameraState& c_, void* out_, hipStream_t s_) : e(e_), c(c_), out(out_), stream(s_), cur(s_), mode(c_.desc.mode), pseed(pass_seed(e_.base_seed, c_.frame, SEED_GI_PREVIEW)) {}
    uint32_t seed(uint32_t pass) const { return pass_seed(e.base_seed, c.frame, pass); }
    auto gi_preview_src() const { return s.gi_source == 0 ? a.gi_res[1] : a.gi_res[2]; }
    double slot_bytes(int slot) const {
        const KernelInfo& ki = kernel_info(slot);
        const uint32_t cols = c.col1 - c.col0;
        return (double)(c.row1 - c.row0) * (ki.half ? (double)(((cols + 7u) / 8u / 2u) * 8u) : (double)cols) * ki.bytes_per_unit;
    }
    template <class F> void run(int slot, uint64_t bits, F&& launch, double own_bytes = -1.0) {
        if (e.last_launches.empty() || e.last_launches.back() != bits) e.last_launches.push_back(bits);
        if ((bits & e.pass_mask) != bits) { mask_split |= (bits & e.pass_mask) != 0; return; }
        if (e.launch_filter != ~0ull && !((e.launch_filter >> (launch_ordinal++ & 63u)) & 1ull)) return;
        const double bytes = own_bytes >= 0.0 ? own_bytes : slot_bytes(slot);
        a.ray_counter = c.counters.as<unsigned long long>() + kCounterWordsPerSlot * slot;
        if (e.profiling && e.profile_kernel_events) {
            (void)e.profile_close();
            g_launch_events.start = e.take_event(); g_launch_events.stop = e.take_event(); g_launch_events.consumed = false;
            launch();
            if (g_launch_events.consumed) e.profile_records.push_back({slot, g_launch_events.start, g_launch_events.stop, bytes, 1u, true});
            else { e.event_pool.push_back(g_launch_events.start); e.event_pool.push_back(g_launch_events.stop); }
            g_launch_events = LaunchEvents();
            return;
        }
        const bool atrous = slot == KS_DENOISE_WAVELET || slot == KS_DENOISE_WAVELET_12 || slot == KS_DENOISE_WAVELET_COMPOSE;
        e.profile_begin(e.profile_group_atrous && atrous ? (int)KS_DENOISE_WAVELET_FAMILY : slot, cur, bytes);
        launch();
    }
    bool node_wanted(int n) const {
        const bool perspective = c.has_gbuffer() && dof_perspective(c.desc.projection);
        switch (n) {
        case kNodeFog: return c.fog.on && perspective;
        case kNodeShafts: return c.shafts.on && perspective;
        case kNodeDof: return c.dof.on && perspective;
        case kNodeMBlur: return c.mblur.on && c.has_gbuffer();
        case kNodeGrade: return c.grade.on && c.desc.mode != ST_MODE_BVH_HEATMAP;
        case kNodeLens: return c.lens.on && c.desc.mode != ST_MODE_BVH_HEATMAP;
        default: return c.bloom.on && c.desc.mode != ST_MODE_BVH_HEATMAP;
        }
    }
    template <int N> int node_planes(int n, FencedPlanes<N>& p, const size_t (&bytes)[N]) {
        if (int rc = p.acquire(bytes, p.Grow, stream)) return rc;
        route.hdr_plane[n] = p.plane[0].ptr; route.planes_read[n] = &p.read;
        return ST_OK;
    }
    int node_plan(int n) {
        const uint32_t w = c.desc.width, h = c.desc.height;
        const size_t plane = (size_t)w * h * sizeof(float4);
        switch (n) {
        case kNodeFog: return node_planes(n, c.fog.planes, {plane});
        case kNodeShafts:
            if (int rc = Engine::shafts_plan(c.shafts.desc, w, h, work.shafts_plan)) return rc;
            return node_planes(n, c.shafts.planes, {plane, work.shafts_plan.cell_bytes});
        case kNodeDof:
            if (int rc = Engine::dof_plan(c.dof.desc, w, h, work.dof_plan)) return rc;
            return node_planes(n, c.dof.planes, {plane, work.dof_plan.packed_bytes, work.dof_plan.tile_bytes, work.dof_plan.tile_bytes});
        case kNodeMBlur:
            if (int rc = Engine::mblur_plan(c.mblur.desc, w, h, work.mblur_plan)) return rc;
            return node_planes(n, c.mblur.planes, {plane, work.mblur_plan.packed_bytes, work.mblur_plan.tile_bytes, work.mblur_plan.tile_bytes});
        case kNodeLens:
            if (int rc = Engine::lens_plan(c.lens.desc, w, h, work.lens_plan)) return rc;
            return node_planes(n, c.lens.planes, {plane});
        case kNodeGrade:
            if (int rc = Engine::grade_plan(c.grade.desc, work.grade_plan)) return rc;
            work.grade_lut = e.live_lut(c.grade.desc.lut);
            return node_planes(n, c.grade.planes, {plane});
        default:
            if (int rc = Engine::bloom_plan(c.bloom.desc, w, h, work.bloom_plan)) return rc;
            if (work.bloom_plan.levels == 0u) return ST_OK;
            return node_planes(n, c.bloom.planes, {plane, work.bloom_plan.texels * sizeof(float4)});
        }
    }
    void node_arm(int n, const NodeTarget& t) {
        const NodeSource src{route.hdr_plane[n], a.g0, a.velocity, true, c.desc.width, c.desc.height};
        const float sun[3] = {e.sun_dir_.x, e.sun_dir_.y, e.sun_dir_.z};
        const NodeView view{c.desc.transform, c.desc.projection, sun};
        switch (n) {
        case kNodeFog: Engine::fog_step(c.fog.desc, view, src, c.row0, c.row1, c.col0, c.col1, t, work.fog); break;
        case kNodeShafts: e.shafts_steps(c.shafts.desc, work.shafts_plan, view, src, c.shafts.planes.plane[1].as<float4>(), t, true, work.shafts); break;
        case kNodeDof: { const auto& p = c.dof.planes.plane; Engine::dof_steps(c.dof.desc, work.dof_plan, c.desc.projection, src, p[1].as<float2>(), p[2].as<float>(), p[3].as<float>(), t, work.dof); break; }
        case kNodeLens: Engine::lens_step(c.lens.desc, work.lens_plan, src, c.frame, e.lens_force_gather, t, work.lens); break;
        case kNodeGrade:
            Engine::grade_step(c.grade.desc, work.grade_plan, work.grade_lut ? work.grade_lut->texels.as<float4>() : nullptr, work.grade_lut ? work.grade_lut->size : 0u, src,
                               c.row0, c.row1, c.col0, c.col1, t, work.grade);
// ... 67 lines not shown
        a.sm = P(alt ? ST_BUF_PRIM_SURFACE_MAP_B : ST_BUF_PRIM_SURFACE_MAP_A); a.psm = P(alt ? ST_BUF_PRIM_SURFACE_MAP_A : ST_BUF_PRIM_SURFACE_MAP_B);
        a.sn = P(ST_BUF_COUNT + (alt ? 1 : 0)); a.psn = P(ST_BUF_COUNT + (alt ? 0 : 1));
        a.reprojection = P(ST_BUF_REPROJECTION_MAP); a.velocity = P(ST_BUF_VELOCITY_MAP);
        for (int i = 0; i < 3; i++) a.di_res[i] = P(ST_BUF_DI_RESERVOIRS_0 + i);
        a.di_diff_samples = P(ST_BUF_DI_DIFF_SAMPLES); a.di_diff_prev_colors = P(ST_BUF_DI_DIFF_PREV_COLORS); a.di_diff_curr_colors = P(ST_BUF_DI_DIFF_CURR_COLORS);
        a.di_diff_moments = P(alt ? ST_BUF_DI_DIFF_MOMENTS_B : ST_BUF_DI_DIFF_MOMENTS_A); a.di_diff_prev_moments = P(alt ? ST_BUF_DI_DIFF_MOMENTS_A : ST_BUF_DI_DIFF_MOMENTS_B);
        a.di_diff_stash = P(ST_BUF_DI_DIFF_STASH); a.di_spec_samples = P(ST_BUF_DI_SPEC_SAMPLES);
        a.gi_d0 = P(ST_BUF_GI_D0); a.gi_d1 = P(ST_BUF_GI_D1); a.gi_d2 = P(ST_BUF_GI_D2);
        for (int i = 0; i < 4; i++) a.gi_res[i] = P(ST_BUF_GI_RESERVOIRS_0 + i);
        a.gi_diff_samples = P(ST_BUF_GI_DIFF_SAMPLES); a.gi_diff_prev_colors = P(ST_BUF_GI_DIFF_PREV_COLORS); a.gi_diff_curr_colors = P(ST_BUF_GI_DIFF_CURR_COLORS);
        a.gi_diff_moments = P(alt ? ST_BUF_GI_DIFF_MOMENTS_B : ST_BUF_GI_DIFF_MOMENTS_A); a.gi_diff_prev_moments = P(alt ? ST_BUF_GI_DIFF_MOMENTS_A : ST_BUF_GI_DIFF_MOMENTS_B);
        a.gi_diff_stash = P(ST_BUF_GI_DIFF_STASH); a.gi_spec_samples = P(ST_BUF_GI_SPEC_SAMPLES);
        a.ref_hits = P(ST_BUF_REF_HITS); a.ref_rays = P(ST_BUF_REF_RAYS); a.ref_colors = P(ST_BUF_REF_COLORS);
        a.dbg_used_memory = reinterpret_cast<uint32_t*>(P(ST_BUF_DBG_USED_MEMORY));
        a.width = c.desc.width; a.height = c.desc.height; a.row0 = c.row0; a.row1 = c.row1; a.col0 = c.col0; a.col1 = c.col1;
        a.frame = c.frame; a.tile_map = e.tuning.tile_map;
        return ST_OK;
    }
    int decide_switches() {
        e.last_launches.clear();
        if (mode != ST_MODE_BVH_HEATMAP && mode != ST_MODE_REFERENCE) {
            a.tile_mask = c.tile_mask.as<unsigned long long>();
            a.gi_late_mask = a.tile_mask ? a.tile_mask + c.tile_mask_tiles() : nullptr;
        }
        const StTuning& t = e.tuning; const bool fast = e.arithmetic == ST_ARITH_FAST;
        s.needs_di = mode == ST_MODE_IMAGE || mode == ST_MODE_DI_DIFFUSE || mode == ST_MODE_DI_SPECULAR;
        s.needs_gi = mode == ST_MODE_IMAGE || mode == ST_MODE_GI_DIFFUSE || mode == ST_MODE_GI_SPECULAR;
        s.denoise = c.desc.denoise != 0u; s.any_objects = !e.instances.records.empty();
        s.tracing = c.frame % 6u < 4u; s.gi_source = (s.tracing && c.frame % 2u == 1u) ? 1u : 0u;
        s.whole_graph = e.pass_mask == ~0ull;
        s.gi_runs = s.needs_gi && s.any_objects;
        if (c.gi_aliased && s.gi_runs && !s.whole_graph) if (int rc = materialize_gi_history(c)) return rc;
        s.swap_gi_history = t.alias_gi_history && fast && s.gi_runs && s.whole_graph && s.gi_source == 0u;
        if (s.gi_runs && s.whole_graph) c.gi_aliased = false;
        s.gi_skip_history_copy = s.swap_gi_history ? 1u : 0u;
        s.gi_preview_both = t.preview_both && s.whole_graph && t.fuse && s.gi_runs && a.gi_late_mask;
        s.even_tiles = (((a.width + 7u) / 8u) & 1u) == 0u;
        const bool fused_denoised = s.whole_graph && t.fuse && s.denoise && s.any_objects;
        s.variance_in_reproject = (t.variance_in_reproject && fused_denoised && t.fuse_wavelet && s.needs_di && s.needs_gi && a.tile_mask) ? 1u : 0u;
        if (t.lean_frame && fast && fused_denoised && mode == ST_MODE_IMAGE) {
            s.lean = kLeanPrim | kLeanSamples;
            if (t.fuse_gi_reprojection && s.tracing && s.even_tiles && (c.frame % 2u == 0u || a.width % 2u == 0u)) s.lean |= kLeanGiRes2;
            if (s.gi_preview_both) s.lean |= kLeanGiMid;
            if (route.keep_velocity) s.lean |= kLeanKeepVelocity;
        }
        s.compose_in_wavelet = t.fuse_compose && fast && fused_denoised && out != nullptr && mode == ST_MODE_IMAGE;
        s.skip_dead_scratch = (t.skip_scratch_stores && fused_denoised && t.fuse_spatial && s.even_tiles && s.needs_di) ? 1u : 0u;
        s.fuse_gi_validation_now = t.fuse && t.fuse_gi_reprojection && t.fuse_gi_sampling && t.fuse_gi_validation && !s.tracing && s.whole_graph;
        s.fuse_gi_reprojection_now = (t.fuse && t.fuse_gi_reprojection && s.tracing) || s.fuse_gi_validation_now;
        s.two_streams = t.overlap && !e.profiling && e.launch_filter == ~0ull && s.needs_di && s.needs_gi && s.any_objects;
        a.gi_skip_history_copy = s.gi_skip_history_copy; a.variance_in_reproject = s.variance_in_reproject; a.lean = s.lean; a.skip_dead_scratch = s.skip_dead_scratch;
        c.last_lean = s.lean; c.last_lean_composed = s.compose_in_wavelet && s.lean != 0u;
        return ST_OK;
    }
    void arm_output() {
        for (int n = 0; n < kHdrNodes; n++) if (route.on(n)) node_arm(n, route.target(n));
    }
    void refresh_inputs() {
        if (c.surface_map_replaced[0] || c.surface_map_replaced[1]) {
            const uint32_t now = c.frame % 2u == 1u ? 1u : 0u;
            e.L.launch_refresh_internal_planes(a, (c.surface_map_replaced[now] ? 1u : 0u) | (c.surface_map_replaced[now ^ 1u] ? 2u : 0u), stream);
            c.surface_map_replaced[0] = c.surface_map_replaced[1] = false; luts_generated_now = true;
        }
        if (mode == ST_MODE_BVH_HEATMAP) return;
        if (!e.atmosphere_initialized) {
            e.L.launch_atmosphere_static(static_cast<float4*>(e.d_transmittance.ptr), static_cast<float4*>(e.d_scattering.ptr), stream);
            e.atmosphere_initialized = true; luts_generated_now = true;
        }
        if (!e.sky_known || e.known_sun_altitude != e.sun_altitude) {
            e.L.launch_atmosphere_sky(static_cast<const float4*>(e.d_transmittance.ptr), static_cast<const float4*>(e.d_scattering.ptr), e.sun_altitude, static_cast<float4*>(e.d_sky.ptr), stream);
            e.sky_known = true; e.known_sun_altitude = e.sun_altitude; luts_generated_now = true;
        }
    }
    void observer_modes() {
        if (mode == ST_MODE_BVH_HEATMAP) { run(KS_BVH_HEATMAP, ST_PASS_BVH_HEATMAP, [&] { e.L.launch_bvh_heatmap(a, cur); }); return; }
        for (uint32_t d = 0; d <= c.desc.depth; d++) {
            run(KS_REF_TRACING, ST_PASS_REF_TRACING, [&] { e.L.launch_ref_tracing(a, d, cur); });
            run(KS_REF_SHADING, ST_PASS_REF_SHADING, [&] { e.L.launch_ref_shading(a, seed(SEED_REF_SHADING + d), d, cur); });
        }
        run(KS_REF_SHADING, ST_PASS_REF_SHADING, [&] { e.L.launch_ref_shading(a, seed(SEED_REF_SHADING + 255u), 255u, cur); });
    }
    void prim() {
        (void)c.gbuffer_depth_read[c.frame % 2u].wait(cur, Fence::OtherStreams, Fence::Clear);
        if (e.tuning.fuse && s.any_objects) run(KS_PRIM_VISIBILITY_REPROJECTION, ST_PASS_PRIM_VISIBILITY | ST_PASS_FRAME_REPROJECTION, [&] { e.L.launch_prim_visibility(a, true, e.deform.deform_table(), e.deform.deform_posed(), nm_tri_geo, cur); });
        else run(KS_PRIM_VISIBILITY, ST_PASS_PRIM_VISIBILITY, [&] { e.L.launch_prim_visibility(a, false, e.deform.deform_table(), e.deform.deform_posed(), nm_tri_geo, cur); });
        if (s.any_objects && !e.tuning.fuse) run(KS_FRAME_REPROJECTION, ST_PASS_FRAME_REPROJECTION, [&] { e.L.launch_frame_reprojection(a, cur); });
    }
    void di_head() {
        if (e.tuning.fuse && e.tuning.fuse_di_head) run(KS_DI_SAMPLING_TEMPORAL, ST_PASS_DI_SAMPLING | ST_PASS_DI_TEMPORAL, [&] { e.L.launch_di_sampling_temporal(a, seed(SEED_DI_SAMPLING), seed(SEED_DI_TEMPORAL), cur); });
        else {
            run(KS_DI_SAMPLING, ST_PASS_DI_SAMPLING, [&] { e.L.launch_di_sampling(a, seed(SEED_DI_SAMPLING), cur); });
            run(KS_DI_TEMPORAL, ST_PASS_DI_TEMPORAL, [&] { e.L.launch_di_temporal(a, seed(SEED_DI_TEMPORAL), cur); });
        }
    }
    void di_tail() {
        const StTuning& t = e.tuning;
        if (t.fuse && t.fuse_spatial && s.even_tiles) run(KS_DI_SPATIAL_FUSED, ST_PASS_DI_SPATIAL_PICK | ST_PASS_DI_SPATIAL_TRACE | ST_PASS_DI_SPATIAL_SAMPLE, [&] { e.L.launch_di_spatial_fused(a, seed(SEED_DI_SPATIAL_PICK), seed(SEED_DI_SPATIAL_SAMPLE), cur); });
        else {
            run(KS_DI_SPATIAL_PICK, ST_PASS_DI_SPATIAL_PICK, [&] { e.L.launch_di_spatial_pick(a, seed(SEED_DI_SPATIAL_PICK), cur); });
            run(KS_DI_SPATIAL_TRACE, ST_PASS_DI_SPATIAL_TRACE, [&] { e.L.launch_spatial_trace(a, a.di_diff_samples, a.di_diff_curr_colors, a.di_diff_stash, cur); });
            run(KS_DI_SPATIAL_SAMPLE, ST_PASS_DI_SPATIAL_SAMPLE, [&] { e.L.launch_di_spatial_sample(a, seed(SEED_DI_SPATIAL_SAMPLE), cur); });
        }
        if (t.fuse && s.denoise) { run(KS_DI_RESOLVING_REPROJECT, ST_PASS_DI_RESOLVING | ST_PASS_DENOISE_REPROJECT_DI, [&] { e.L.launch_di_resolving(a, true, cur); }); di_reprojected = true; }
        else run(KS_DI_RESOLVING, ST_PASS_DI_RESOLVING, [&] { e.L.launch_di_resolving(a, false, cur); });
    }
    void gi_temporal() {
        if (s.fuse_gi_reprojection_now) run(KS_GI_REPROJECTION_TEMPORAL, ST_PASS_GI_REPROJECTION | ST_PASS_GI_TEMPORAL, [&] { e.L.launch_gi_temporal(a, seed(SEED_GI_TEMPORAL), true, cur); });
        else run(KS_GI_TEMPORAL, ST_PASS_GI_TEMPORAL, [&] { e.L.launch_gi_temporal(a, seed(SEED_GI_TEMPORAL), false, cur); });
    }
    void gi_sampling() {
        if (e.tuning.fuse && e.tuning.fuse_gi_sampling) { run(KS_GI_SAMPLING_AB, ST_PASS_GI_SAMPLING_A | ST_PASS_GI_SAMPLING_B, [&] { e.L.launch_gi_sampling_ab(a, seed(SEED_GI_SAMPLING_A), seed(SEED_GI_SAMPLING_B), s.fuse_gi_validation_now, cur); }); return; }
        run(KS_GI_SAMPLING_A, ST_PASS_GI_SAMPLING_A, [&] { e.L.launch_gi_sampling_a(a, seed(SEED_GI_SAMPLING_A), cur); });
        run(KS_GI_SAMPLING_B, ST_PASS_GI_SAMPLING_B, [&] { e.L.launch_gi_sampling_b(a, seed(SEED_GI_SAMPLING_B), cur); });
    }
    void gi_head() {
        if (!s.fuse_gi_reprojection_now) run(KS_GI_REPROJECTION, ST_PASS_GI_REPROJECTION, [&] { e.L.launch_gi_reprojection(a, cur); });
        if (s.tracing) {
            if (c.frame % 2u == 0u) gi_sampling();
            gi_temporal();
            if (c.frame % 2u == 1u) {
                if (e.tuning.fuse && e.tuning.fuse_spatial && s.even_tiles)
                    run(KS_GI_SPATIAL_FUSED, ST_PASS_GI_SPATIAL_PICK | ST_PASS_GI_SPATIAL_TRACE | ST_PASS_GI_SPATIAL_SAMPLE, [&] { e.L.launch_gi_spatial_fused(a, seed(SEED_GI_SPATIAL_PICK), seed(SEED_GI_SPATIAL_SAMPLE), cur); });
                else {
                    run(KS_GI_SPATIAL_PICK, ST_PASS_GI_SPATIAL_PICK, [&] { e.L.launch_gi_spatial_pick(a, seed(SEED_GI_SPATIAL_PICK), cur); });
                    run(KS_GI_SPATIAL_TRACE, ST_PASS_GI_SPATIAL_TRACE, [&] { e.L.launch_spatial_trace(a, a.gi_d0, a.gi_d1, a.gi_d2, cur); });
                    run(KS_GI_SPATIAL_SAMPLE, ST_PASS_GI_SPATIAL_SAMPLE, [&] { e.L.launch_gi_spatial_sample(a, seed(SEED_GI_SPATIAL_SAMPLE), cur); });
                }
            }
        } else { gi_sampling(); gi_temporal(); }
        if (!s.gi_preview_both) run(KS_GI_PREVIEW, ST_PASS_GI_PREVIEW_0, [&] { e.L.launch_gi_preview(a, pseed, 0u, gi_preview_src(), a.gi_res[3], cur); });
    }
    void gi_tail() {
        const bool dn = s.denoise; const uint32_t gi_source = s.gi_source;
        if (s.gi_preview_both) {
            const uint64_t group = ST_PASS_GI_PREVIEW_0 | ST_PASS_GI_PREVIEW_1 | ST_PASS_GI_RESOLVING | (dn ? (uint64_t)ST_PASS_DENOISE_REPROJECT_GI : 0ull);
            run(dn ? KS_GI_PREVIEW_BOTH : KS_GI_PREVIEW_BOTH_NO_REPROJECT, group, [&] { e.L.launch_gi_preview_both(a, pseed, gi_preview_src(), a.gi_res[3], gi_source, dn, cur); });
            a.gi_preview_late = 1u;
            a.gi_mid_src = (a.lean & kLeanGiMid) ? gi_preview_src() : nullptr;
            run(KS_GI_PREVIEW_LATE, group, [&] { e.L.launch_gi_preview_resolve(a, pseed, 1u, a.gi_res[3], gi_source, dn, cur); });
            a.gi_preview_late = 0u; a.gi_mid_src = nullptr;
            if (dn) gi_reprojected = true;
        } else if (e.tuning.fuse) {
            if (dn) { run(KS_GI_PREVIEW_RESOLVE_REPROJECT, ST_PASS_GI_PREVIEW_1 | ST_PASS_GI_RESOLVING | ST_PASS_DENOISE_REPROJECT_GI, [&] { e.L.launch_gi_preview_resolve(a, pseed, 1u, a.gi_res[3], gi_source, true, cur); }); gi_reprojected = true; }
            else run(KS_GI_PREVIEW_RESOLVE, ST_PASS_GI_PREVIEW_1 | ST_PASS_GI_RESOLVING, [&] { e.L.launch_gi_preview_resolve(a, pseed, 1u, a.gi_res[3], gi_source, false, cur); });
        } else {
            run(KS_GI_PREVIEW, ST_PASS_GI_PREVIEW_1, [&] { e.L.launch_gi_preview(a, pseed, 1u, a.gi_res[3], a.gi_res[0], cur); });
            run(KS_GI_RESOLVING, ST_PASS_GI_RESOLVING, [&] { e.L.launch_gi_resolving(a, gi_source, cur); });
        }
        if (s.swap_gi_history) { std::swap(c.plane[ST_BUF_GI_RESERVOIRS_0], c.plane[ST_BUF_GI_RESERVOIRS_1]); c.gi_aliased = true; }
    }
    void denoise() {
        if (!s.denoise) return;
        struct MapScope { KArgs& a; uint32_t saved; MapScope(KArgs& a_, uint32_t m) : a(a_), saved(a_.tile_map) { a.tile_map = m; } ~MapScope() { a.tile_map = saved; } } map_scope(a, e.tuning.tile_map_denoise);
        if (!di_reprojected) run(KS_DENOISE_REPROJECT, ST_PASS_DENOISE_REPROJECT_DI, [&] { e.L.launch_denoise_reproject(a, a.di_diff_prev_colors, a.di_diff_prev_moments, a.di_diff_samples, a.di_diff_curr_colors, a.di_diff_moments, cur); });
        if (!gi_reprojected) run(KS_DENOISE_REPROJECT, ST_PASS_DENOISE_REPROJECT_GI, [&] { e.L.launch_denoise_reproject(a, a.gi_diff_prev_colors, a.gi_diff_prev_moments, a.gi_diff_samples, a.gi_diff_curr_colors, a.gi_diff_moments, cur); });
        float4* di[3] = {a.di_diff_stash, a.di_diff_prev_colors, a.di_diff_curr_colors};
        float4* gi[3] = {a.gi_diff_stash, a.gi_diff_prev_colors, a.gi_diff_curr_colors};
        const int in_ix[5] = {0, 1, 0, 2, 0}, out_ix[5] = {1, 0, 2, 0, 2};
        uint32_t first = 0;
        auto side_point = [&](uint32_t point) {
            if (!s.two_streams || first != 2u || e.tuning.side_start != point) return;
            side_rc = c.ev_lds_done.record(stream); c.have_lds_done = side_rc == ST_OK;
        };
        if (e.tuning.fuse && e.tuning.fuse_wavelet) {
            const uint64_t group = ST_PASS_DENOISE_VARIANCE | ST_PASS_DENOISE_WAVELET_0 | ((uint64_t)ST_PASS_DENOISE_WAVELET_0 << 1);
            float4* tmp_di = a.variance_in_reproject ? a.di_diff_curr_colors : c.plane[ST_BUF_COUNT + 2];
            float4* tmp_gi = a.variance_in_reproject ? a.gi_diff_curr_colors : c.plane[ST_BUF_COUNT + 3];
            run(KS_DENOISE_VARIANCE, group, [&] { e.L.launch_denoise_variance(a, tmp_di, tmp_gi, cur); });
            run(KS_DENOISE_WAVELET_12, group, [&] { e.L.launch_denoise_wavelet_12(a, 1.0f, 2.0f, tmp_di, di[1], di[0], tmp_gi, gi[1], gi[0], cur); });
            first = 2;
            side_point(1u);
        } else run(KS_DENOISE_VARIANCE, ST_PASS_DENOISE_VARIANCE, [&] { e.L.launch_denoise_variance(a, a.di_diff_stash, a.gi_diff_stash, cur); });
        for (uint32_t nth = first; nth < 5; nth++) {
            if (nth == 4u && s.compose_in_wavelet) {
                Engine::present_guard(c, out, cur); e.dist_guard(c.handle, out, cur);
                run(KS_DENOISE_WAVELET_COMPOSE, ((uint64_t)ST_PASS_DENOISE_WAVELET_0 << nth) | ST_PASS_COMPOSITION, [&] {
                    e.L.launch_denoise_wavelet_compose(a, 1u << nth, (float)(1u + nth), di[in_ix[nth]], di[out_ix[nth]], gi[in_ix[nth]], gi[out_ix[nth]], mode, route.comp_out, route.comp_format, a.lean == 0u, route.comp_disp, cur); });
                composed = true;
                continue;
            }
            run(KS_DENOISE_WAVELET, (uint64_t)ST_PASS_DENOISE_WAVELET_0 << nth, [&] { e.L.launch_denoise_wavelet(a, 1u << nth, (float)(1u + nth), di[in_ix[nth]], di[out_ix[nth]], gi[in_ix[nth]], gi[out_ix[nth]], cur); });
            side_point(nth);
        }
    }
    void pack_early() {
        for (int n = 0; n < kHdrNodes; n++) if (route.on(n)) run_node(n, 0u, kHdrNode[n].early);
    }
    void compose() {
        if (!out || composed) return;
        Engine::present_guard(c, out, cur); e.dist_guard(c.handle, out, cur);
        const bool dn = s.denoise;
        const float4* di_diff = (dn && (mode == ST_MODE_IMAGE || mode == ST_MODE_DI_DIFFUSE)) ? a.di_diff_curr_colors : a.di_diff_samples;
        const float4* gi_diff = (dn && (mode == ST_MODE_IMAGE || mode == ST_MODE_GI_DIFFUSE)) ? a.gi_diff_curr_colors : a.gi_diff_samples;
        run(KS_COMPOSITION, ST_PASS_COMPOSITION, [&] { e.L.launch_composition(a, mode, di_diff, gi_diff, route.comp_out, route.comp_format, route.comp_disp, cur); });
        composed = true;
    }

    int two_streams() {
        const StTuning& t = e.tuning;
        if (!c.side_stream) {
            int least = 0, greatest = 0;
            (void)hipDeviceGetStreamPriorityRange(&least, &greatest);
            const int priority = t.side_priority > 0 ? greatest : (t.side_priority < 0 ? least : 0);
            ST_HIP(hipStreamCreateWithPriority(&c.side_stream.h, hipStreamNonBlocking, priority));
        }
        if (luts_generated_now) { if (int rc = c.ev_setup.record(stream)) return rc; if (int rc = c.ev_setup.wait(c.side_stream)) return rc; }
        if (int rc = e.copies.begin(c.side_stream, kReadsNothing)) return rc;
        if (c.have_prev_frame_events) { if (int rc = c.ev_prim_ok.wait(c.side_stream)) return rc; }
        if (c.have_prev_frame_events && c.have_lds_done) { if (int rc = c.ev_lds_done.wait(c.side_stream)) return rc; }
        c.have_lds_done = false;
        cur = c.side_stream;
        prim();
        if (!t.di_head_on_main) di_head();
        if (int rc = c.ev_di_head.record(c.side_stream)) return rc;
        gi_head();
        if (c.have_prev_frame_events) { if (int rc = c.ev_frame_done.wait(c.side_stream)) return rc; }
        gi_tail();
        if (int rc = c.ev_gi_done.record(c.side_stream)) return rc;
        cur = stream;
        if (int rc = c.ev_di_head.wait(stream)) return rc;
        if (t.di_head_on_main) di_head();
        di_tail();
        pack_early();
        const bool reproject_later = s.denoise && !t.fuse;
        if (!reproject_later) { if (int rc = c.ev_prim_ok.record(stream)) return rc; }
        if (int rc = c.ev_gi_done.wait(stream)) return rc;
        denoise();
        if (side_rc) return side_rc;
        if (reproject_later) { if (int rc = c.ev_prim_ok.record(stream)) return rc; }
        compose();
        if (int rc = c.ev_frame_done.record(stream)) return rc;
        c.have_prev_frame_events = true;
        return ST_OK;
    }
    int serial() {
        if (mode == ST_MODE_BVH_HEATMAP || mode == ST_MODE_REFERENCE) { observer_modes(); compose(); return ST_OK; }
        prim();
        if (s.any_objects) {
            if (s.needs_di) { di_head(); di_tail(); }
            if (s.needs_gi) { gi_head(); gi_tail(); }
        }
        pack_early();
        denoise();
        compose();
        c.have_lds_done = false;
        if (c.side_stream) { if (int rc = c.ev_prim_ok.record(stream)) return rc; if (int rc = c.ev_frame_done.record(stream)) return rc; }
        return ST_OK;
    }
    int finish_output() {
        cur = stream;
        int last_depth_reader = -1;
        for (int n = 0; n < kHdrNodes; n++) if (route.on(n) && kHdrNode[n].reads_depth) last_depth_reader = n;
        for (int n = 0; n < kHdrNodes; n++) {
            if (!route.on(n)) continue;
            run_node(n, kHdrNode[n].early, node_steps(n));
            if (int rc = route.planes_read[n]->record(stream)) return rc;
            if (n == kNodeGrade && work.grade_lut) if (int rc = work.grade_lut->fence.record(stream)) return rc;
            if (n == last_depth_reader) if (int rc = c.gbuffer_depth_read[c.frame % 2u].record(stream)) return rc;
        }
        if (route.post) {
            void* const composed = c.post.planes.plane[0].ptr; void* const fxaa_out = c.post.planes.plane[1].ptr;
            const uint32_t w = c.desc.width, h = c.desc.height;
            const bool up = route.up_steps;
            if (route.up_nearest) {
                StPostDesc nearest{}; nearest.output_width = c.upscale.desc.output_width; nearest.output_height = c.upscale.desc.output_height; nearest.filter = ST_RESAMPLE_NEAREST;
                const Engine::PostPlan plan = Engine::post_plan(nearest, false, composed, w, h, nullptr, out, c.out_format);
                run(KS_POST_RESAMPLE, ST_PASS_POST, [&] { e.L.launch_post_resample(plan.rs, cur); }, plan.resample_bytes);
            } else if (route.post_fxaa || !up) {
                const Engine::PostPlan plan = Engine::post_plan(c.post.desc, route.post_fxaa, composed, w, h, fxaa_out, up ? fxaa_out : out, up ? (uint32_t)ST_FORMAT_RGBA32F : c.out_format);
                if (plan.fxaa) run(KS_POST_FXAA, ST_PASS_POST, [&] { e.L.launch_post_fxaa(plan.fx, cur); }, plan.fxaa_bytes);
                if (plan.resample) run(KS_POST_RESAMPLE, ST_PASS_POST, [&] { e.L.launch_post_resample(plan.rs, cur); }, plan.resample_bytes);
            }
            if (up) {
                const Engine::UpscalePlan plan = Engine::upscale_plan(c.upscale.desc, route.post_fxaa ? fxaa_out : composed, w, h, c.upscale.planes.plane[0].ptr, out, c.out_format, e.upscale_fused);
                if (plan.fused) run(KS_UPSCALE_SHARPEN, ST_PASS_POST, [&] { e.L.launch_upscale_sharpen(plan.fu, plan.fused, cur); }, plan.fused_bytes);
                else if (plan.upscale) run(KS_UPSCALE, ST_PASS_POST, [&] { e.L.launch_upscale(plan.up, cur); }, plan.upscale_bytes);
                if (plan.sharpen && !plan.fused) run(KS_SHARPEN, ST_PASS_POST, [&] { e.L.launch_sharpen(plan.sh, cur); }, plan.sharpen_bytes);
                if (int rc = c.upscale.planes.done(stream)) return rc;
            }
            if (int rc = c.post.planes.done(stream)) return rc;
        }
        if (route.comp_disp.meter && out) if (int rc = e.display_finalize(c, stream)) return rc;
        return ST_OK;
    }
};
}

int Engine::render(CameraState& c, void* out, hipStream_t stream) {
    if (!has_device) return fail(ST_ERR_NO_DEVICE, "render_camera on a host-only engine");
    if (!copies.scene.written) return fail(ST_ERR_INVALID_ARGUMENT, "st_tick must precede st_render_camera");
    ST_HIP(hipSetDevice(device));
    if (int rc = copies.begin(stream, kReadsFrame)) return rc;
    Frame f(*this, c, out, stream);
    if (int rc = f.route_output()) return rc;
    if (int rc = f.bind_args()) return rc;
    f.refresh_inputs();
    if (int rc = f.decide_switches()) return rc;
    f.arm_output();
    if (int rc = f.s.two_streams ? f.two_streams() : f.serial()) return rc;
    if (int rc = f.finish_output()) return rc;
    if (int rc = copies.end(stream, kReadsFrame)) return rc;
    profile_close();
    ST_HIP(hipGetLastError());
    if (f.mask_split) return fail(ST_ERR_INVALID_ARGUMENT, "the pass mask splits a fused launch (st_debug_last_launches lists the launch groups)");
    return ST_OK;
}

}
```

strolle_amd/csrc/st_types.h:

```cpp
#pragma once
#include "st_math.h"

namespace st {

struct GpuCamera {
    M4 projection_view;
    M4 ndc_to_world;
    float4 origin;
    float4 screen;
};
static_assert(sizeof(GpuCamera) == 160, "Camera uniform is 160 B");

struct GpuMaterial {
    float4 base_color, base_color_texture, emissive, emissive_texture;
    float roughness, metallic, reflectance, ior;
    float4 metallic_roughness_texture, normal_map_texture;
};
static_assert(sizeof(GpuMaterial) == 112, "Material is 112 B");

struct GpuLight { float4 d0, d1, d2, d3, prev_d0, prev_d1, prev_d2; };
static_assert(sizeof(GpuLight) == 112, "Light is 112 B");

struct HostTriangle { float4 d0, d1, d2, d3, d4, d5, d6, d7, d8; };
static_assert(sizeof(HostTriangle) == 144, "Triangle is 144 B");

constexpr uint32_t kRefitBatch = 512;
constexpr uint32_t kLeanPrim = 1u;
constexpr uint32_t kLeanSamples = 2u;
constexpr uint32_t kLeanGiRes2 = 4u;
constexpr uint32_t kLeanGiMid = 8u;
constexpr uint32_t kLeanKeepVelocity = 16u;
constexpr int kBvhStackSize = 24;
constexpr int kBvhStackSizeDeep = 32;
constexpr uint32_t kLightIdSky = 0xffffffffu;
constexpr uint32_t kLdsSceneTexels = 448;
constexpr uint32_t kLdsLights = 16;
constexpr uint32_t kCounterLines = 256;

struct EnvCell { float q; uint32_t alias; float p; };
static_assert(sizeof(EnvCell) == 12, "an importance cell is 12 B");

constexpr uint32_t kDisplayBins = 64;
constexpr uint32_t kDisplayRaw = 0xffffffffu;
struct DisplayArgs {
    uint32_t on, tonemap, meter;
    float scale;
    const float* state;
    uint32_t* hist;
    float ev_min, bins_per_ev;
};
constexpr uint32_t kDisplayReplicas = 64;
struct DisplayState { float scale, metered_ev, adapted_ev; uint32_t primed, frames, pad[3]; };
static_assert(sizeof(DisplayState) == 32, "the display state is 32 B");
constexpr size_t kDisplayLastOffset = (size_t)kDisplayReplicas * kDisplayBins * sizeof(uint32_t);
constexpr size_t kDisplayStateOffset = kDisplayLastOffset + kDisplayBins * sizeof(uint32_t);
constexpr size_t kDisplayBytes = kDisplayStateOffset + sizeof(DisplayState);

struct PostArgs {
    const float4* src; void* dst;
    uint32_t width, height, out_width, out_height, format, filter;
    float edge_threshold, edge_threshold_min, subpixel;
};

struct UpscaleArgs {
    const float4* src; void* dst;
    uint32_t width, height, out_width, out_height, format, denoise;
    float sharpness;
};

struct BloomArgs {
    const float4* src; void* dst; const float4* base;
    uint32_t sw, sh, dw, dh, format, additive, firefly, threshold_on;
    float factor, clamp, threshold, knee_lo , knee2 , knee_div ;
    DisplayArgs display;
};

struct BloomTailArgs {
    float4* base; uint32_t bw, bh, n, additive, lds_bytes;
    uint32_t w[8], h[8], off[8];
    float factor[8];
};

constexpr uint32_t kMBlurTile = 32u;
struct MBlurArgs {
// ... 118 lines not shown
```

Measured before the change: 10030.

## Alternate tile sweep direction between consecutive passes for cache reuse

```diff
diff --git a/include/strolle_hip.h b/include/strolle_hip.h
--- a/include/strolle_hip.h
+++ b/include/strolle_hip.h
@@ -506,6 +506,7 @@
 };
 int st_debug_set_pass_mask(StEngine* e, uint64_t mask);
 int st_debug_set_launch_filter(StEngine* e, uint64_t filter);
+int st_debug_set_sweep(StEngine* e, int sweep, uint32_t* in_force);
 int st_debug_variance_flags(StEngine* e, StHandle camera, uint64_t* tile_mask_out, size_t capacity_tiles, size_t* tiles);
 int st_debug_last_launches(StEngine* e, uint64_t* out_bits, size_t capacity, size_t* count);
 int st_camera_ray_count(StEngine* e, StHandle camera, uint64_t* out, int reset);
diff --git a/rust/strolle-hip/src/ffi.rs b/rust/strolle-hip/src/ffi.rs
--- a/rust/strolle-hip/src/ffi.rs
+++ b/rust/strolle-hip/src/ffi.rs
@@ -168,6 +168,7 @@
     pub fn st_debug_device_tree_refits(e: *mut StEngine, ticks: *mut u64) -> i32;
     pub fn st_engine_get_tuning(e: *mut StEngine, out: *mut StTuning) -> i32;
     pub fn st_engine_set_tuning(e: *mut StEngine, tuning: *const StTuning) -> i32;
+    pub fn st_debug_set_sweep(e: *mut StEngine, sweep: i32, in_force: *mut u32) -> i32;
     pub fn st_camera_set_window(e: *mut StEngine, camera: u64, x0: u32, y0: u32, x1: u32, y1: u32) -> i32;
     pub fn st_dist_partition(width: u32, height: u32, world: u32, cols: u32, rank: u32, owned: *mut StDistRect) -> i32;
     pub fn st_dist_window(width: u32, height: u32, owned: *const StDistRect, apron: u32, window: *mut StDistRect) -> i32;
diff --git a/strolle_amd/api.py b/strolle_amd/api.py
--- a/strolle_amd/api.py
+++ b/strolle_amd/api.py
@@ -730,6 +730,8 @@
             self.camera_write_buffer = fn("camera_write_buffer", [vp, u64, i32, vp, sz])
             self.debug_set_pass_mask = fn("debug_set_pass_mask", [vp, u64]); self.debug_set_launch_filter = fn("debug_set_launch_filter", [vp, u64]); self.debug_last_launches = fn("debug_last_launches", [vp, P(u64), sz, P(sz)])
             self.debug_keep_all_planes = fn("debug_keep_all_planes", [vp, i32])
+            if hasattr(lib, prefix + "debug_set_sweep"):
+                self.debug_set_sweep = fn("debug_set_sweep", [vp, i32, P(u32)])
             self.camera_buffer_stale = fn("camera_buffer_stale", [vp, u64, i32, P(i32)])
             self.camera_present_copy = fn("camera_present_copy", [vp, u64, vp, vp, sz, vp])
             self.camera_present_ready = fn("camera_present_ready", [vp, u64, vp, i32, P(i32)])
@@ -1016,6 +1018,11 @@
     def set_launch_filter(self, mask: int):
         self._check(self._b.debug_set_launch_filter(self._h, mask & 0xFFFFFFFFFFFFFFFF))
 
+    def set_sweep(self, sweep: int = -1) -> int:
+        in_force = C.c_uint32(0)
+        self._check(self._b.debug_set_sweep(self._h, int(sweep), C.byref(in_force)))
+        return int(in_force.value)
+
     def last_launches(self):
         arr = (C.c_uint64 * 64)(); n = C.c_size_t()
         self._check(self._b.debug_last_launches(self._h, arr, 64, C.byref(n)))
diff --git a/strolle_amd/csrc/k_common.h b/strolle_amd/csrc/k_common.h
--- a/strolle_amd/csrc/k_common.h
+++ b/strolle_amd/csrc/k_common.h
@@ -14,19 +14,7 @@
 #define ST_STACK_LDS(SE, name) extern __shared__ __align__(16) unsigned char st_stack_lds_[]; SE* name = reinterpret_cast<SE*>(st_stack_lds_)
 inline uint32_t stack_lds_bytes(const KArgs& a, size_t slot_bytes) { return a.stack_entries * (uint32_t)kBlockThreads * (uint32_t)slot_bytes; }
 
-struct TileWindow { uint32_t tx0, tx1, ty0, ty1; };
-__host__ __device__ inline TileWindow tile_window(const KArgs& a, bool half_x) {
-    uint32_t tiles_x = (a.width + 7u) >> 3;
-    if (half_x) tiles_x >>= 1;
-    const uint32_t shift = half_x ? 4u : 3u, round = half_x ? 15u : 7u;
-    TileWindow w;
-    w.tx0 = a.col0 >> shift;
-    w.tx1 = (a.col1 + round) >> shift; if (w.tx1 > tiles_x) w.tx1 = tiles_x;
-    if (w.tx0 > w.tx1) w.tx0 = w.tx1;
-    w.ty0 = a.row0 >> 3;
-    w.ty1 = (a.row1 + 7u) >> 3;
-    return w;
-}
+__host__ __device__ inline TileWindow tile_window(const KArgs& a, bool half_x) { return tile_window_of(a.width, a.row0, a.row1, a.col0, a.col1, half_x); }
 struct LaunchDims { uint32_t tiles_x, tile_x0, tile_y0, tile_y1, blocks; };
 inline LaunchDims launch_dims(const KArgs& a, bool half_x) {
     const TileWindow w = tile_window(a, half_x);
diff --git a/strolle_amd/csrc/k_denoise.hip b/strolle_amd/csrc/k_denoise.hip
--- a/strolle_amd/csrc/k_denoise.hip
+++ b/strolle_amd/csrc/k_denoise.hip
@@ -197,27 +197,14 @@
 constexpr int kWvW = 32, kWvH = 16, kWvThreads = kWvW * kWvH;
 struct WaveletBlock { int32_t x0, y0; bool valid; };
 __host__ __device__ inline void wavelet_grid(const KArgs& a, uint32_t bw, uint32_t* bx0, uint32_t* groups_x, uint32_t* rows) {
-    const uint32_t c1 = a.col1 < a.width ? a.col1 : a.width;
-    *bx0 = a.col0 / bw;
-    const uint32_t bx1 = (c1 + bw - 1u) / bw;
-    *groups_x = bx1 > *bx0 ? bx1 - *bx0 : 0u;
-    const uint32_t ty0 = a.row0 >> 3, ty1 = (a.row1 + 7u) >> 3;
-    *rows = ((ty1 - ty0) * 8u + kWvH - 1u) / kWvH;
+    wavelet_grid_of(a.width, a.row0, a.row1, a.col0, a.col1, bw, (uint32_t)kWvH, bx0, groups_x, rows);
 }
 template <int BW = kWvW>
 ST_D WaveletBlock wavelet_block(const KArgs& a) {
     uint32_t bx0, groups_x, rows;
     wavelet_grid(a, BW, &bx0, &groups_x, &rows);
     const uint32_t ty0 = a.row0 >> 3;
-    const uint32_t n_blocks = groups_x * rows, b = blockIdx.x;
-    uint32_t lin = b;
-    if (a.tile_map == 0u) {
-        const uint32_t q = n_blocks >> 3, r = n_blocks & 7u, xcd = b & 7u, k = b >> 3;
-        lin = (xcd < r ? xcd * (q + 1u) : r * (q + 1u) + (xcd - r) * q) + k;
-    } else if (a.tile_map == 2u) {
-        const uint32_t chunk = groups_x * 2u * 8u, full = (n_blocks / chunk) * chunk;
-        if (b < full) { const uint32_t c = b / chunk, i = b - c * chunk; lin = c * chunk + (i & 7u) * (groups_x * 2u) + (i >> 3); }
-    }
+    const uint32_t lin = block_linear(blockIdx.x, groups_x, groups_x * rows, kWaveletChunkRows, a.tile_map);
     WaveletBlock w;
     const uint32_t gy = lin / groups_x, gx = lin - gy * groups_x;
     w.x0 = (int32_t)((bx0 + gx) * BW); w.y0 = (int32_t)(ty0 * 8u + gy * kWvH);
diff --git a/strolle_amd/csrc/st_abi.cpp b/strolle_amd/csrc/st_abi.cpp
--- a/strolle_amd/csrc/st_abi.cpp
+++ b/strolle_amd/csrc/st_abi.cpp
@@ -513,6 +513,13 @@
     E(e)->launch_filter = filter;
     return ST_OK;
 }
+int st_debug_set_sweep(StEngine* e, int sweep, uint32_t* in_force) {
+    ST_REQUIRE(e, "null engine");
+    ST_REQUIRE(sweep >= -1 && sweep <= 2, "sweep is 0, 1 or 2 (-1: no change)");
+    if (sweep >= 0) E(e)->sweep = (uint32_t)sweep;
+    if (in_force) *in_force = E(e)->sweep;
+    return ST_OK;
+}
 int st_debug_last_launches(StEngine* e, uint64_t* out_bits, size_t capacity, size_t* count) {
     ST_REQUIRE(e && count, "null argument");
     const std::vector<uint64_t>& v = E(e)->last_launches;
diff --git a/strolle_amd/csrc/st_device.h b/strolle_amd/csrc/st_device.h
--- a/strolle_amd/csrc/st_device.h
+++ b/strolle_amd/csrc/st_device.h
@@ -9,20 +9,7 @@
 ST_D TileCoord tile_for_block(uint32_t b, uint32_t tiles_x, uint32_t tiles_y, uint32_t map_mode) {
     const uint32_t groups_x = (tiles_x + 3u) >> 2;
     const uint32_t n_blocks = groups_x * tiles_y;
-    uint32_t lin = b;
-    if (map_mode == 0u) {
-        const uint32_t q = n_blocks >> 3, r = n_blocks & 7u;
-        const uint32_t xcd = b & 7u, k = b >> 3;
-        lin = (xcd < r ? xcd * (q + 1u) : r * (q + 1u) + (xcd - r) * q) + k;
-    } else if (map_mode == 2u) {
-        const uint32_t chunk = groups_x * 4u * 8u;
-        const uint32_t full = (n_blocks / chunk) * chunk;
-        if (b < full) {
-            const uint32_t c = b / chunk, i = b - c * chunk;
-            const uint32_t xcd = i & 7u, k = i >> 3;
-            lin = c * chunk + xcd * (groups_x * 4u) + k;
-        }
-    }
+    const uint32_t lin = block_linear(b, groups_x, n_blocks, kTileChunkRows, map_mode);
     const uint32_t wave = threadIdx.x >> 6;
     TileCoord t;
     t.y = lin / groups_x;
diff --git a/strolle_amd/csrc/st_engine.cpp b/strolle_amd/csrc/st_engine.cpp
--- a/strolle_amd/csrc/st_engine.cpp
+++ b/strolle_amd/csrc/st_engine.cpp
@@ -49,6 +49,7 @@
     staging.enabled = tuning.staging != 0u;
     if (const char* x = getenv("ST_BLOOM_TAIL_BYTES")) bloom_tail_wanted = atoi(x);
     if (const char* x = getenv("ST_UPSCALE_FUSED")) upscale_fused = (uint32_t)atoi(x) <= 3u ? (uint32_t)atoi(x) : 0u;
+    if (const char* x = getenv("ST_SWEEP")) sweep = (uint32_t)atoi(x) <= 2u ? (uint32_t)atoi(x) : 0u;
     if (const char* x = getenv("ST_EXP")) exp_flags = (uint32_t)strtoul(x, nullptr, 0);
     if (const char* ex = getenv("ST_EXACT")) if (atoi(ex) != 0) { arithmetic = ST_ARITH_EXACT; L = launchers_exact(); }
 }
diff --git a/strolle_amd/csrc/st_engine.h b/strolle_amd/csrc/st_engine.h
--- a/strolle_amd/csrc/st_engine.h
+++ b/strolle_amd/csrc/st_engine.h
@@ -420,6 +420,7 @@
     uint64_t launch_filter = ~0ull;
     uint64_t pass_mask = ~0ull;
     StTuning tuning;
+    uint32_t sweep = 1u;
     uint32_t exp_flags = 0;
     bool profiling = false;
     bool count_bytes = false;
diff --git a/strolle_amd/csrc/st_render.cpp b/strolle_amd/csrc/st_render.cpp
--- a/strolle_amd/csrc/st_render.cpp
+++ b/strolle_amd/csrc/st_render.cpp
@@ -162,6 +162,12 @@
     const uint32_t mode, pseed;
     bool mask_split = false, di_reprojected = false, gi_reprojected = false, composed = false, luts_generated_now = false; uint32_t launch_ordinal = 0u;
     int side_rc = ST_OK;
+    bool di_rev = true, gi_rev = true, atrous_rev = false;
+    void sweep(bool reversed, bool atrous = false) {
+        const bool on = e.sweep == 1u || (atrous && e.sweep == 2u);
+        a.tile_map = tile_map_mode(a.tile_map) | (on && reversed ? kTileMapReverse : 0u);
+    }
+    void turn(bool& reversed, bool atrous = false) { sweep(reversed, atrous); reversed = !reversed; }
     Frame(Engine& e_, CameraState& c_, void* out_, hipStream_t s_) : e(e_), c(c_), out(out_), stream(s_), cur(s_), mode(c_.desc.mode), pseed(pass_seed(e_.base_seed, c_.frame, SEED_GI_PREVIEW)) {}
     uint32_t seed(uint32_t pass) const { return pass_seed(e.base_seed, c.frame, pass); }
     auto gi_preview_src() const { return s.gi_source == 0 ? a.gi_res[1] : a.gi_res[2]; }
@@ -395,56 +401,60 @@
     }
     void prim() {
         (void)c.gbuffer_depth_read[c.frame % 2u].wait(cur, Fence::OtherStreams, Fence::Clear);
+        sweep(false);
         if (e.tuning.fuse && s.any_objects) run(KS_PRIM_VISIBILITY_REPROJECTION, ST_PASS_PRIM_VISIBILITY | ST_PASS_FRAME_REPROJECTION, [&] { e.L.launch_prim_visibility(a, true, e.deform.deform_table(), e.deform.deform_posed(), nm_tri_geo, cur); });
         else run(KS_PRIM_VISIBILITY, ST_PASS_PRIM_VISIBILITY, [&] { e.L.launch_prim_visibility(a, false, e.deform.deform_table(), e.deform.deform_posed(), nm_tri_geo, cur); });
         if (s.any_objects && !e.tuning.fuse) run(KS_FRAME_REPROJECTION, ST_PASS_FRAME_REPROJECTION, [&] { e.L.launch_frame_reprojection(a, cur); });
     }
     void di_head() {
-        if (e.tuning.fuse && e.tuning.fuse_di_head) run(KS_DI_SAMPLING_TEMPORAL, ST_PASS_DI_SAMPLING | ST_PASS_DI_TEMPORAL, [&] { e.L.launch_di_sampling_temporal(a, seed(SEED_DI_SAMPLING), seed(SEED_DI_TEMPORAL), cur); });
+        if (e.tuning.fuse && e.tuning.fuse_di_head) { turn(di_rev); run(KS_DI_SAMPLING_TEMPORAL, ST_PASS_DI_SAMPLING | ST_PASS_DI_TEMPORAL, [&] { e.L.launch_di_sampling_temporal(a, seed(SEED_DI_SAMPLING), seed(SEED_DI_TEMPORAL), cur); }); }
         else {
-            run(KS_DI_SAMPLING, ST_PASS_DI_SAMPLING, [&] { e.L.launch_di_sampling(a, seed(SEED_DI_SAMPLING), cur); });
-            run(KS_DI_TEMPORAL, ST_PASS_DI_TEMPORAL, [&] { e.L.launch_di_temporal(a, seed(SEED_DI_TEMPORAL), cur); });
+            turn(di_rev); run(KS_DI_SAMPLING, ST_PASS_DI_SAMPLING, [&] { e.L.launch_di_sampling(a, seed(SEED_DI_SAMPLING), cur); });
+            turn(di_rev); run(KS_DI_TEMPORAL, ST_PASS_DI_TEMPORAL, [&] { e.L.launch_di_temporal(a, seed(SEED_DI_TEMPORAL), cur); });
         }
     }
     void di_tail() {
         const StTuning& t = e.tuning;
-        if (t.fuse && t.fuse_spatial && s.even_tiles) run(KS_DI_SPATIAL_FUSED, ST_PASS_DI_SPATIAL_PICK | ST_PASS_DI_SPATIAL_TRACE | ST_PASS_DI_SPATIAL_SAMPLE, [&] { e.L.launch_di_spatial_fused(a, seed(SEED_DI_SPATIAL_PICK), seed(SEED_DI_SPATIAL_SAMPLE), cur); });
+        if (t.fuse && t.fuse_spatial && s.even_tiles) { turn(di_rev); run(KS_DI_SPATIAL_FUSED, ST_PASS_DI_SPATIAL_PICK | ST_PASS_DI_SPATIAL_TRACE | ST_PASS_DI_SPATIAL_SAMPLE, [&] { e.L.launch_di_spatial_fused(a, seed(SEED_DI_SPATIAL_PICK), seed(SEED_DI_SPATIAL_SAMPLE), cur); }); }
         else {
-            run(KS_DI_SPATIAL_PICK, ST_PASS_DI_SPATIAL_PICK, [&] { e.L.launch_di_spatial_pick(a, seed(SEED_DI_SPATIAL_PICK), cur); });
-            run(KS_DI_SPATIAL_TRACE, ST_PASS_DI_SPATIAL_TRACE, [&] { e.L.launch_spatial_trace(a, a.di_diff_samples, a.di_diff_curr_colors, a.di_diff_stash, cur); });
-            run(KS_DI_SPATIAL_SAMPLE, ST_PASS_DI_SPATIAL_SAMPLE, [&] { e.L.launch_di_spatial_sample(a, seed(SEED_DI_SPATIAL_SAMPLE), cur); });
-        }
+            turn(di_rev); run(KS_DI_SPATIAL_PICK, ST_PASS_DI_SPATIAL_PICK, [&] { e.L.launch_di_spatial_pick(a, seed(SEED_DI_SPATIAL_PICK), cur); });
+            turn(di_rev); run(KS_DI_SPATIAL_TRACE, ST_PASS_DI_SPATIAL_TRACE, [&] { e.L.launch_spatial_trace(a, a.di_diff_samples, a.di_diff_curr_colors, a.di_diff_stash, cur); });
+            turn(di_rev); run(KS_DI_SPATIAL_SAMPLE, ST_PASS_DI_SPATIAL_SAMPLE, [&] { e.L.launch_di_spatial_sample(a, seed(SEED_DI_SPATIAL_SAMPLE), cur); });
+        }
+        turn(di_rev);
         if (t.fuse && s.denoise) { run(KS_DI_RESOLVING_REPROJECT, ST_PASS_DI_RESOLVING | ST_PASS_DENOISE_REPROJECT_DI, [&] { e.L.launch_di_resolving(a, true, cur); }); di_reprojected = true; }
         else run(KS_DI_RESOLVING, ST_PASS_DI_RESOLVING, [&] { e.L.launch_di_resolving(a, false, cur); });
     }
     void gi_temporal() {
+        turn(gi_rev);
         if (s.fuse_gi_reprojection_now) run(KS_GI_REPROJECTION_TEMPORAL, ST_PASS_GI_REPROJECTION | ST_PASS_GI_TEMPORAL, [&] { e.L.launch_gi_temporal(a, seed(SEED_GI_TEMPORAL), true, cur); });
         else run(KS_GI_TEMPORAL, ST_PASS_GI_TEMPORAL, [&] { e.L.launch_gi_temporal(a, seed(SEED_GI_TEMPORAL), false, cur); });
     }
     void gi_sampling() {
-        if (e.tuning.fuse && e.tuning.fuse_gi_sampling) { run(KS_GI_SAMPLING_AB, ST_PASS_GI_SAMPLING_A | ST_PASS_GI_SAMPLING_B, [&] { e.L.launch_gi_sampling_ab(a, seed(SEED_GI_SAMPLING_A), seed(SEED_GI_SAMPLING_B), s.fuse_gi_validation_now, cur); }); return; }
-        run(KS_GI_SAMPLING_A, ST_PASS_GI_SAMPLING_A, [&] { e.L.launch_gi_sampling_a(a, seed(SEED_GI_SAMPLING_A), cur); });
-        run(KS_GI_SAMPLING_B, ST_PASS_GI_SAMPLING_B, [&] { e.L.launch_gi_sampling_b(a, seed(SEED_GI_SAMPLING_B), cur); });
+        if (e.tuning.fuse && e.tuning.fuse_gi_sampling) { turn(gi_rev); run(KS_GI_SAMPLING_AB, ST_PASS_GI_SAMPLING_A | ST_PASS_GI_SAMPLING_B, [&] { e.L.launch_gi_sampling_ab(a, seed(SEED_GI_SAMPLING_A), seed(SEED_GI_SAMPLING_B), s.fuse_gi_validation_now, cur); }); return; }
+        turn(gi_rev); run(KS_GI_SAMPLING_A, ST_PASS_GI_SAMPLING_A, [&] { e.L.launch_gi_sampling_a(a, seed(SEED_GI_SAMPLING_A), cur); });
+        turn(gi_rev); run(KS_GI_SAMPLING_B, ST_PASS_GI_SAMPLING_B, [&] { e.L.launch_gi_sampling_b(a, seed(SEED_GI_SAMPLING_B), cur); });
     }
     void gi_head() {
-        if (!s.fuse_gi_reprojection_now) run(KS_GI_REPROJECTION, ST_PASS_GI_REPROJECTION, [&] { e.L.launch_gi_reprojection(a, cur); });
+        if (!s.fuse_gi_reprojection_now) { turn(gi_rev); run(KS_GI_REPROJECTION, ST_PASS_GI_REPROJECTION, [&] { e.L.launch_gi_reprojection(a, cur); }); }
         if (s.tracing) {
             if (c.frame % 2u == 0u) gi_sampling();
             gi_temporal();
             if (c.frame % 2u == 1u) {
-                if (e.tuning.fuse && e.tuning.fuse_spatial && s.even_tiles)
-                    run(KS_GI_SPATIAL_FUSED, ST_PASS_GI_SPATIAL_PICK | ST_PASS_GI_SPATIAL_TRACE | ST_PASS_GI_SPATIAL_SAMPLE, [&] { e.L.launch_gi_spatial_fused(a, seed(SEED_GI_SPATIAL_PICK), seed(SEED_GI_SPATIAL_SAMPLE), cur); });
-                else {
-                    run(KS_GI_SPATIAL_PICK, ST_PASS_GI_SPATIAL_PICK, [&] { e.L.launch_gi_spatial_pick(a, seed(SEED_GI_SPATIAL_PICK), cur); });
-                    run(KS_GI_SPATIAL_TRACE, ST_PASS_GI_SPATIAL_TRACE, [&] { e.L.launch_spatial_trace(a, a.gi_d0, a.gi_d1, a.gi_d2, cur); });
-                    run(KS_GI_SPATIAL_SAMPLE, ST_PASS_GI_SPATIAL_SAMPLE, [&] { e.L.launch_gi_spatial_sample(a, seed(SEED_GI_SPATIAL_SAMPLE), cur); });
+                if (e.tuning.fuse && e.tuning.fuse_spatial && s.even_tiles) {
+                    turn(gi_rev); run(KS_GI_SPATIAL_FUSED, ST_PASS_GI_SPATIAL_PICK | ST_PASS_GI_SPATIAL_TRACE | ST_PASS_GI_SPATIAL_SAMPLE, [&] { e.L.launch_gi_spatial_fused(a, seed(SEED_GI_SPATIAL_PICK), seed(SEED_GI_SPATIAL_SAMPLE), cur); });
+                } else {
+                    turn(gi_rev); run(KS_GI_SPATIAL_PICK, ST_PASS_GI_SPATIAL_PICK, [&] { e.L.launch_gi_spatial_pick(a, seed(SEED_GI_SPATIAL_PICK), cur); });
+                    turn(gi_rev); run(KS_GI_SPATIAL_TRACE, ST_PASS_GI_SPATIAL_TRACE, [&] { e.L.launch_spatial_trace(a, a.gi_d0, a.gi_d1, a.gi_d2, cur); });
+                    turn(gi_rev); run(KS_GI_SPATIAL_SAMPLE, ST_PASS_GI_SPATIAL_SAMPLE, [&] { e.L.launch_gi_spatial_sample(a, seed(SEED_GI_SPATIAL_SAMPLE), cur); });
                 }
             }
         } else { gi_sampling(); gi_temporal(); }
-        if (!s.gi_preview_both) run(KS_GI_PREVIEW, ST_PASS_GI_PREVIEW_0, [&] { e.L.launch_gi_preview(a, pseed, 0u, gi_preview_src(), a.gi_res[3], cur); });
+        if (!s.gi_preview_both) { turn(gi_rev); run(KS_GI_PREVIEW, ST_PASS_GI_PREVIEW_0, [&] { e.L.launch_gi_preview(a, pseed, 0u, gi_preview_src(), a.gi_res[3], cur); }); }
     }
     void gi_tail() {
         const bool dn = s.denoise; const uint32_t gi_source = s.gi_source;
+        sweep(true);
         if (s.gi_preview_both) {
             const uint64_t group = ST_PASS_GI_PREVIEW_0 | ST_PASS_GI_PREVIEW_1 | ST_PASS_GI_RESOLVING | (dn ? (uint64_t)ST_PASS_DENOISE_REPROJECT_GI : 0ull);
             run(dn ? KS_GI_PREVIEW_BOTH : KS_GI_PREVIEW_BOTH_NO_REPROJECT, group, [&] { e.L.launch_gi_preview_both(a, pseed, gi_preview_src(), a.gi_res[3], gi_source, dn, cur); });
@@ -457,14 +467,15 @@
             if (dn) { run(KS_GI_PREVIEW_RESOLVE_REPROJECT, ST_PASS_GI_PREVIEW_1 | ST_PASS_GI_RESOLVING | ST_PASS_DENOISE_REPROJECT_GI, [&] { e.L.launch_gi_preview_resolve(a, pseed, 1u, a.gi_res[3], gi_source, true, cur); }); gi_reprojected = true; }
             else run(KS_GI_PREVIEW_RESOLVE, ST_PASS_GI_PREVIEW_1 | ST_PASS_GI_RESOLVING, [&] { e.L.launch_gi_preview_resolve(a, pseed, 1u, a.gi_res[3], gi_source, false, cur); });
         } else {
-            run(KS_GI_PREVIEW, ST_PASS_GI_PREVIEW_1, [&] { e.L.launch_gi_preview(a, pseed, 1u, a.gi_res[3], a.gi_res[0], cur); });
-            run(KS_GI_RESOLVING, ST_PASS_GI_RESOLVING, [&] { e.L.launch_gi_resolving(a, gi_source, cur); });
+            sweep(false); run(KS_GI_PREVIEW, ST_PASS_GI_PREVIEW_1, [&] { e.L.launch_gi_preview(a, pseed, 1u, a.gi_res[3], a.gi_res[0], cur); });
+            sweep(true); run(KS_GI_RESOLVING, ST_PASS_GI_RESOLVING, [&] { e.L.launch_gi_resolving(a, gi_source, cur); });
         }
         if (s.swap_gi_history) { std::swap(c.plane[ST_BUF_GI_RESERVOIRS_0], c.plane[ST_BUF_GI_RESERVOIRS_1]); c.gi_aliased = true; }
     }
     void denoise() {
         if (!s.denoise) return;
         struct MapScope { KArgs& a; uint32_t saved; MapScope(KArgs& a_, uint32_t m) : a(a_), saved(a_.tile_map) { a.tile_map = m; } ~MapScope() { a.tile_map = saved; } } map_scope(a, e.tuning.tile_map_denoise);
+        sweep(true);
         if (!di_reprojected) run(KS_DENOISE_REPROJECT, ST_PASS_DENOISE_REPROJECT_DI, [&] { e.L.launch_denoise_reproject(a, a.di_diff_prev_colors, a.di_diff_prev_moments, a.di_diff_samples, a.di_diff_curr_colors, a.di_diff_moments, cur); });
         if (!gi_reprojected) run(KS_DENOISE_REPROJECT, ST_PASS_DENOISE_REPROJECT_GI, [&] { e.L.launch_denoise_reproject(a, a.gi_diff_prev_colors, a.gi_diff_prev_moments, a.gi_diff_samples, a.gi_diff_curr_colors, a.gi_diff_moments, cur); });
         float4* di[3] = {a.di_diff_stash, a.di_diff_prev_colors, a.di_diff_curr_colors};
@@ -479,12 +490,13 @@
             const uint64_t group = ST_PASS_DENOISE_VARIANCE | ST_PASS_DENOISE_WAVELET_0 | ((uint64_t)ST_PASS_DENOISE_WAVELET_0 << 1);
             float4* tmp_di = a.variance_in_reproject ? a.di_diff_curr_colors : c.plane[ST_BUF_COUNT + 2];
             float4* tmp_gi = a.variance_in_reproject ? a.gi_diff_curr_colors : c.plane[ST_BUF_COUNT + 3];
-            run(KS_DENOISE_VARIANCE, group, [&] { e.L.launch_denoise_variance(a, tmp_di, tmp_gi, cur); });
-            run(KS_DENOISE_WAVELET_12, group, [&] { e.L.launch_denoise_wavelet_12(a, 1.0f, 2.0f, tmp_di, di[1], di[0], tmp_gi, gi[1], gi[0], cur); });
+            turn(atrous_rev, true); run(KS_DENOISE_VARIANCE, group, [&] { e.L.launch_denoise_variance(a, tmp_di, tmp_gi, cur); });
+            turn(atrous_rev, true); run(KS_DENOISE_WAVELET_12, group, [&] { e.L.launch_denoise_wavelet_12(a, 1.0f, 2.0f, tmp_di, di[1], di[0], tmp_gi, gi[1], gi[0], cur); });
             first = 2;
             side_point(1u);
-        } else run(KS_DENOISE_VARIANCE, ST_PASS_DENOISE_VARIANCE, [&] { e.L.launch_denoise_variance(a, a.di_diff_stash, a.gi_diff_stash, cur); });
+        } else { turn(atrous_rev, true); run(KS_DENOISE_VARIANCE, ST_PASS_DENOISE_VARIANCE, [&] { e.L.launch_denoise_variance(a, a.di_diff_stash, a.gi_diff_stash, cur); }); }
         for (uint32_t nth = first; nth < 5; nth++) {
+            turn(atrous_rev, true);
             if (nth == 4u && s.compose_in_wavelet) {
                 Engine::present_guard(c, out, cur); e.dist_guard(c.handle, out, cur);
                 run(KS_DENOISE_WAVELET_COMPOSE, ((uint64_t)ST_PASS_DENOISE_WAVELET_0 << nth) | ST_PASS_COMPOSITION, [&] {
@@ -497,9 +509,11 @@
         }
     }
     void pack_early() {
+        sweep(false);
         for (int n = 0; n < kHdrNodes; n++) if (route.on(n)) run_node(n, 0u, kHdrNode[n].early);
     }
     void compose() {
+        sweep(false);
         if (!out || composed) return;
         Engine::present_guard(c, out, cur); e.dist_guard(c.handle, out, cur);
         const bool dn = s.denoise;
@@ -561,7 +575,7 @@
         return ST_OK;
     }
     int finish_output() {
-        cur = stream;
+        cur = stream; sweep(false);
         int last_depth_reader = -1;
         for (int n = 0; n < kHdrNodes; n++) if (route.on(n) && kHdrNode[n].reads_depth) last_depth_reader = n;
         for (int n = 0; n < kHdrNodes; n++) {
diff --git a/strolle_amd/csrc/st_tile_map.h b/strolle_amd/csrc/st_tile_map.h
--- /dev/null
+++ b/strolle_amd/csrc/st_tile_map.h
@@ -0,0 +1,66 @@
+#pragma once
+#include <cstdint>
+
+#if defined(__HIPCC__)
+#define ST_MAP_FN __host__ __device__ __forceinline__
+#else
+#define ST_MAP_FN inline
+#endif
+
+namespace st {
+
+constexpr uint32_t kTileMapReverse = 1u << 31;
+ST_MAP_FN uint32_t tile_map_mode(uint32_t map_word) { return map_word & ~kTileMapReverse; }
+
+ST_MAP_FN uint32_t sweep_reversed(uint32_t b, uint32_t n_blocks) {
+    if (b >= n_blocks) return b;
+    const uint32_t r = b & 7u, last = (n_blocks - 1u - r) >> 3;
+    return r + ((last - (b >> 3)) << 3);
+}
+
+ST_MAP_FN uint32_t block_linear(uint32_t b, uint32_t groups_x, uint32_t n_blocks, uint32_t chunk_rows, uint32_t map_word) {
+    const uint32_t b_reversed = sweep_reversed(b, n_blocks);
+    b = (map_word & kTileMapReverse) ? b_reversed : b;
+    const uint32_t map_mode = tile_map_mode(map_word);
+    uint32_t lin = b;
+    if (map_mode == 0u) {
+        const uint32_t q = n_blocks >> 3, r = n_blocks & 7u;
+        const uint32_t xcd = b & 7u, k = b >> 3;
+        lin = (xcd < r ? xcd * (q + 1u) : r * (q + 1u) + (xcd - r) * q) + k;
+    } else if (map_mode == 2u) {
+        const uint32_t chunk = groups_x * chunk_rows * 8u;
+        const uint32_t full = (n_blocks / chunk) * chunk;
+        if (b < full) {
+            const uint32_t c = b / chunk, i = b - c * chunk;
+            const uint32_t xcd = i & 7u, k = i >> 3;
+            lin = c * chunk + xcd * (groups_x * chunk_rows) + k;
+        }
+    }
+    return lin;
+}
+constexpr uint32_t kTileChunkRows = 4u;
+constexpr uint32_t kWaveletChunkRows = 2u;
+
+struct TileWindow { uint32_t tx0, tx1, ty0, ty1; };
+ST_MAP_FN TileWindow tile_window_of(uint32_t width, uint32_t row0, uint32_t row1, uint32_t col0, uint32_t col1, bool half_x) {
+    uint32_t tiles_x = (width + 7u) >> 3;
+    if (half_x) tiles_x >>= 1;
+    const uint32_t shift = half_x ? 4u : 3u, round = half_x ? 15u : 7u;
+    TileWindow w;
+    w.tx0 = col0 >> shift;
+    w.tx1 = (col1 + round) >> shift; if (w.tx1 > tiles_x) w.tx1 = tiles_x;
+    if (w.tx0 > w.tx1) w.tx0 = w.tx1;
+    w.ty0 = row0 >> 3;
+    w.ty1 = (row1 + 7u) >> 3;
+    return w;
+}
+ST_MAP_FN void wavelet_grid_of(uint32_t width, uint32_t row0, uint32_t row1, uint32_t col0, uint32_t col1, uint32_t bw, uint32_t bh, uint32_t* bx0, uint32_t* groups_x, uint32_t* rows) {
+    const uint32_t c1 = col1 < width ? col1 : width;
+    *bx0 = col0 / bw;
+    const uint32_t bx1 = (c1 + bw - 1u) / bw;
+    *groups_x = bx1 > *bx0 ? bx1 - *bx0 : 0u;
+    const uint32_t ty0 = row0 >> 3, ty1 = (row1 + 7u) >> 3;
+    *rows = ((ty1 - ty0) * 8u + bh - 1u) / bh;
+}
+
+}
diff --git a/strolle_amd/csrc/st_types.h b/strolle_amd/csrc/st_types.h
--- a/strolle_amd/csrc/st_types.h
+++ b/strolle_amd/csrc/st_types.h
@@ -1,5 +1,6 @@
 #pragma once
 #include "st_math.h"
+#include "st_tile_map.h"
 
 namespace st {
 
```

Measured after the change: 10090, median of 2. About the same (+0.6%).
